# swarth100/dynfu

Hardware: AMD Instinct MI355X
Metric: frames/sec (warp-solve + TSDF fuse), 512^3 vol / 2k nodes / VGA depth (higher is better)
Workload: dtype f32; 1 GPU; C2: 512^3 TSDF, 640x480 depth, 2048 nodes, k=4, 262144 vertices, 5 GN x PCG<=256 (tol 1e-6), reference-parity energy (energy.t), lambda=200; parallelism=replicas x1 (one sequence per GPU, no collective), ranks_seen=1, repeats=5

## Files before the change

dynfu_amd/csrc/capi.cpp:

```cpp
#include <hip/hip_runtime.h>

#include <cmath>
#include <cstdarg>
#include <cstdio>
#include <cstring>
#include <map>
#include <mutex>
#include <new>
#include <utility>
#include <vector>

#include "../../include/dynfu_amd.h"
#include "kernels.hpp"
#include "dev_switch.hpp"
#include "solve.hpp"
#include "solve6.hpp"

namespace {

thread_local char g_err[512] = "";

int fail(int code, const char* fmt, ...) {
    va_list ap;
    va_start(ap, fmt);
// ... 555 lines not shown
int dfa_marching_cubes(const uint32_t* volume, int X, int Y, int Z, const float cell_size[3],
                       const int32_t* tri_table, const int32_t* num_verts_table, float* out_points, int max_vertices,
                       int32_t* total_vertices, dfa_stream_t stream) {
    return marching_cubes_common(volume, X, Y, Z, cell_size, tri_table, num_verts_table, out_points, max_vertices,
                                 total_vertices, nullptr, stream);
}

int dfa_marching_cubes_occ(const uint32_t* volume, const uint8_t* occupancy, int X, int Y, int Z, const float cell_size[3],
                           const int32_t* tri_table, const int32_t* num_verts_table, float* out_points, int max_vertices,
                           int32_t* total_vertices, dfa_stream_t stream) {
    REQUIRE(occupancy, "null occupancy map");
    return marching_cubes_common(volume, X, Y, Z, cell_size, tri_table, num_verts_table, out_points, max_vertices,
                                 total_vertices, occupancy, stream);
}

int dfa_marching_cubes_indexed(const uint32_t* volume, const uint8_t* occupancy, int X, int Y, int Z, const float cell_size[3],
                               const int32_t* tri_table, const int32_t* num_verts_table, float* out_vertices,
                               int max_vertices, int32_t* out_indices, int max_indices, int32_t* totals,
                               dfa_stream_t stream) {
    REQUIRE(volume && X >= 2 && Y >= 2 && Z >= 2, "bad volume");
    REQUIRE(cell_size && tri_table && num_verts_table, "null parameter block / case tables");
    REQUIRE(max_vertices >= 0 && (max_vertices == 0 || out_vertices), "bad vertex buffer");
    REQUIRE(max_indices >= 0 && (max_indices == 0 || out_indices), "bad index buffer");
    REQUIRE(((uintptr_t)out_vertices & 15) == 0, "out_vertices must be 16-byte aligned");
    REQUIRE(totals, "null totals");
    REQUIRE((long)X * Y * Z / 64 < (1L << 31), "volume too large");
    const long nsegs = dfa::mci_segments(X, Y, Z);
    McIndexedScratch& scratch = stream_scratch<McIndexedScratch>(S(stream));
    HIP_TRY(scratch.reserve(nsegs));
    HIP_TRY(dfa::launch_marching_cubes_indexed(volume, X, Y, Z, cell_size, tri_table, num_verts_table, out_vertices,
                                               max_vertices, out_indices, max_indices, totals, scratch.vert.seg_off,
                                               scratch.idx_off, scratch.vert.chunk_sums, occupancy, S(stream)));
    return DFA_OK;
}


static int extract_cloud_common(const uint32_t* volume, int X, int Y, int Z, const float voxel_size[3],
                                const float vol2world[12], float* out_points, int max_points, int32_t* total_points,
                                const uint8_t* occupancy, dfa_stream_t stream) {
    REQUIRE(volume_args_ok(volume, X, Y, Z), "bad volume");
    REQUIRE(voxel_size && vol2world, "null voxel_size / vol2world");
    REQUIRE(max_points >= 0 && (max_points == 0 || out_points), "bad output buffer");
    REQUIRE(((uintptr_t)out_points & 15) == 0, "out_points must be 16-byte aligned");
    REQUIRE((long)X * Y * Z / 64 < (1L << 31), "volume too large");
    const bool vec4  = (X % 4 == 0) && (((uintptr_t)volume & 15) == 0);
    McScratch& scratch = stream_scratch<McScratch>(S(stream));
    HIP_TRY(scratch.reserve(dfa::mc_segments(X, Y, Z, vec4)));
    HIP_TRY(dfa::launch_extract_cloud(volume, X, Y, Z, voxel_size, vol2world, out_points, max_points, total_points,
                                      scratch.seg_off, scratch.chunk_sums, occupancy, S(stream)));
    return DFA_OK;
}

int dfa_tsdf_extract_cloud(const uint32_t* volume, int X, int Y, int Z, const float voxel_size[3], const float vol2world[12],
                           float* out_points, int max_points, int32_t* total_points, dfa_stream_t stream) {
    return extract_cloud_common(volume, X, Y, Z, voxel_size, vol2world, out_points, max_points, total_points, nullptr, stream);
}

int dfa_tsdf_extract_cloud_occ(const uint32_t* volume, const uint8_t* occupancy, int X, int Y, int Z,
                               const float voxel_size[3], const float vol2world[12], float* out_points, int max_points,
                               int32_t* total_points, dfa_stream_t stream) {
    REQUIRE(occupancy, "null occupancy map");
    return extract_cloud_common(volume, X, Y, Z, voxel_size, vol2world, out_points, max_points, total_points, occupancy,
                                stream);
}

int dfa_tsdf_extract_normals(const uint32_t* volume, int X, int Y, int Z, const float voxel_size[3], const float vol2world[12],
                             const float Rinv[9], float gradient_delta_factor, const float* points, int n, float* normals,
                             dfa_stream_t stream) {
    REQUIRE(volume_args_ok(volume, X, Y, Z), "bad volume");
    REQUIRE(voxel_size && vol2world && Rinv, "null voxel_size / vol2world / Rinv");
    REQUIRE(n >= 0 && (n == 0 || (points && normals)), "null points / normals");
    REQUIRE(voxel_size[0] > 0.f && voxel_size[1] > 0.f && voxel_size[2] > 0.f && gradient_delta_factor > 0.f,
            "voxel size and gradient delta must be positive");
    REQUIRE((((uintptr_t)points | (uintptr_t)normals) & 15) == 0, "points / normals must be 16-byte aligned");
    HIP_TRY(dfa::launch_extract_normals(volume, X, Y, Z, voxel_size, vol2world, Rinv, gradient_delta_factor, points, n,
                                        normals, S(stream)));
    return DFA_OK;
}

int dfa_mc_default_tables(int32_t* tri_table, int32_t* num_verts_table) {
    REQUIRE(tri_table && num_verts_table, "null table");
    dfa::mc_default_tables(tri_table, num_verts_table);
    return DFA_OK;
}


int dfa_knn(const float* node_pos, const float* node_w, int D, const float* query, int n_query, int k, int32_t* idx,
            float* weights, dfa_stream_t stream) {
    REQUIRE(node_pos && D > 0, "no nodes");
    REQUIRE(n_query >= 0 && (n_query == 0 || (query && idx)), "bad query / output");
    REQUIRE(k >= 1 && k <= DFA_MAX_KNN, "k out of range 1..16");
    REQUIRE(!weights || node_w, "weights requested without node_w");
    const dfa::KnnGridView* grid = nullptr;
    if (want_grid(D, n_query)) {
        GridScratch& gs = stream_scratch<GridScratch>(S(stream));

        HIP_TRY(gs.reserve(D));

        HIP_TRY(dfa::knn_grid_build(gs.v, node_pos, D, S(stream)));

        grid = &gs.v;
    }
    HIP_TRY(dfa::launch_knn(node_pos, node_w, D, query, n_query, k, idx, weights, grid, S(stream)));
    return DFA_OK;
}

int dfa_warp_to_live(const float* node_pos, const float* node_dq, const float* node_w, int D, int k,
                     const float* vertices, const float* normals, int N, float* out_vertices, float* out_normals,
                     dfa_stream_t stream) {
    REQUIRE(node_pos && node_dq && node_w && D > 0, "no nodes");
    REQUIRE(N >= 0 && (N == 0 || (vertices && out_vertices)), "bad vertices / output");
    REQUIRE(k >= 1 && k <= DFA_MAX_KNN, "k out of range 1..16");
    const dfa::KnnGridView* grid = nullptr;
    if (want_grid(D, N)) {
        GridScratch& gs = stream_scratch<GridScratch>(S(stream));

        HIP_TRY(gs.reserve(D));

        HIP_TRY(dfa::knn_grid_build(gs.v, node_pos, D, S(stream)));

        grid = &gs.v;
    }
    HIP_TRY(dfa::launch_warp_to_live(node_pos, node_dq, node_w, D, k, vertices, normals, N, out_vertices,
                                     out_normals, grid, S(stream)));
    return DFA_OK;
}

int dfa_warp_to_live_graph(const float* node_pos, const float* node_dq, const float* node_w, int D, int k,
                           const int32_t* idx, const float* vertices, const float* normals, int N, float* out_vertices,
                           float* out_normals, dfa_stream_t stream) {
    REQUIRE(node_pos && node_dq && node_w && D > 0, "no nodes");
    REQUIRE(N >= 0 && (N == 0 || (vertices && out_vertices && idx)), "bad vertices / graph / output");
    REQUIRE(k >= 1 && k <= DFA_MAX_KNN, "k out of range 1..16");
    if (N > 0)
        HIP_TRY(dfa::launch_warp_graph(node_pos, node_dq, node_w, k, idx, vertices, normals, N, out_vertices, out_normals,
                                       S(stream)));
    return DFA_OK;
}

int dfa_calc_dqb(const float* node_pos, const float* node_dq, const float* node_w, int D, int k, const float* points,
                 int n, float* out_dq, dfa_stream_t stream) {
    REQUIRE(node_pos && node_dq && node_w && D > 0, "no nodes");
    REQUIRE(n >= 0 && (n == 0 || (points && out_dq)), "bad points / output");
    REQUIRE(k >= 1 && k <= DFA_MAX_KNN, "k out of range 1..16");
    const dfa::KnnGridView* grid = nullptr;
    if (want_grid(D, n)) {
        GridScratch& gs = stream_scratch<GridScratch>(S(stream));

        HIP_TRY(gs.reserve(D));

        HIP_TRY(dfa::knn_grid_build(gs.v, node_pos, D, S(stream)));

        grid = &gs.v;
    }
    HIP_TRY(dfa::launch_dqb_support(node_pos, node_dq, node_w, D, k, points, n, out_dq, nullptr, grid, S(stream)));
    return DFA_OK;
}

int dfa_unsupported_vertices(const float* node_pos, const float* node_w, int D, int k, const float* vertices, int N,
                             uint8_t* flags, dfa_stream_t stream) {
    REQUIRE(N >= 0 && (N == 0 || (vertices && flags)), "bad vertices / output");
    REQUIRE(k >= 1 && k <= DFA_MAX_KNN, "k out of range 1..16");
    if (D == 0) {
        if (N > 0) HIP_TRY(hipMemsetAsync(flags, 1, (size_t)N, S(stream)));
        return DFA_OK;
    }
    REQUIRE(node_pos && node_w && D > 0, "bad nodes");
    const dfa::KnnGridView* grid = nullptr;
    if (want_grid(D, N)) {
        GridScratch& gs = stream_scratch<GridScratch>(S(stream));

        HIP_TRY(gs.reserve(D));

        HIP_TRY(dfa::knn_grid_build(gs.v, node_pos, D, S(stream)));

        grid = &gs.v;
    }
    HIP_TRY(dfa::launch_dqb_support(node_pos, nullptr, node_w, D, k, vertices, N, nullptr, flags, grid, S(stream)));
    return DFA_OK;
}

int dfa_repack_points(const float* src, int src_stride, float* dst, int dst_stride, int n, float pad,
                      dfa_stream_t stream) {
    REQUIRE(n >= 0 && (n == 0 || (src && dst)), "bad points");
    REQUIRE(src_stride >= 3 && dst_stride >= 3, "strides are floats per point, >= 3");
    REQUIRE(src_stride != 4 || ((uintptr_t)src & 15) == 0, "float4 source must be 16-byte aligned");
    REQUIRE(dst_stride != 4 || ((uintptr_t)dst & 15) == 0, "float4 destination must be 16-byte aligned");
    HIP_TRY(dfa::launch_repack_points(src, src_stride, dst, dst_stride, n, pad, S(stream)));
    return DFA_OK;
}

int dfa_transform_points(const float* points, int n, const float aff[12], int with_translation, float* out,
                         dfa_stream_t stream) {
    REQUIRE(n >= 0 && (n == 0 || (points && out)), "bad points");
    REQUIRE(aff, "null transform");
    HIP_TRY(dfa::launch_transform_points(points, n, aff, with_translation != 0, out, S(stream)));
    return DFA_OK;
}

namespace {
struct CompactScratch {
    int32_t* chunks = nullptr;
    int cap         = 0;
    hipError_t reserve(int n_needed) {
        if (n_needed <= cap) return hipSuccess;
        const int n = n_needed + n_needed / 4 + 16;
        (void)hipFree(chunks);
        chunks = nullptr, cap = 0;
        hipError_t e = hipMalloc((void**)&chunks, sizeof(int32_t) * (size_t)n);
        if (e == hipSuccess) cap = n;
        return e;
    }
};
}

int dfa_compact_points(const float* points, const uint8_t* flags, int N, float* out_points, int32_t* out_index,
                       int32_t* count, dfa_stream_t stream) {
    REQUIRE(count, "count is required");
    REQUIRE(N >= 0 && (N == 0 || flags), "bad flags");
    REQUIRE(!out_points || points || N == 0, "out_points requested without points");
    CompactScratch& cs = stream_scratch<CompactScratch>(S(stream));
    HIP_TRY(cs.reserve(dfa::compact_chunks(N > 0 ? N : 1)));
    HIP_TRY(dfa::launch_compact_points(points, flags, N, out_points, out_index, count, cs.chunks, S(stream)));
    return DFA_OK;
}

int dfa_correspond(const float* canon_vertices, const float* canon_normals, int n_canon, const float* live_vertices,
                   int n_live, float* out_vertices, float* out_normals, int32_t* out_index, dfa_stream_t stream) {
    REQUIRE(canon_vertices && n_canon > 0, "no canonical vertices");
    REQUIRE(n_live >= 0 && (n_live == 0 || live_vertices), "bad live vertices");
    REQUIRE(!out_normals || canon_normals, "normals requested without canonical normals");
    const dfa::KnnGridView* grid = nullptr;
    if (n_canon >= 16384 && want_grid(n_canon, n_live)) {
        PointGridScratch& pg = stream_scratch<PointGridScratch>(S(stream));
        HIP_TRY(pg.reserve(n_canon));
        HIP_TRY(dfa::point_grid_build(pg.v, canon_vertices, n_canon, S(stream)));
        grid = &pg.v.g;
    } else if (want_grid(n_canon, n_live)) {
        GridScratch& gs = stream_scratch<GridScratch>(S(stream));

        HIP_TRY(gs.reserve(n_canon));

        HIP_TRY(dfa::knn_grid_build(gs.v, canon_vertices, n_canon, S(stream)));

        grid = &gs.v;
    }
    HIP_TRY(dfa::launch_correspond(canon_vertices, canon_normals, n_canon, live_vertices, n_live, out_vertices,
                                   out_normals, out_index, grid, S(stream)));
    return DFA_OK;
}

int dfa_correspond_projective(const float* vertices, const float* normals, int n, const float* vmap, int vmap_step,
                              const float* nmap, int nmap_step, int cols, int rows, float fx, float fy, float cx, float cy,
                              float dist_thresh, float min_cosine, float* out_vertices, float* out_normals,
                              int32_t* out_pixel, dfa_stream_t stream) {
    REQUIRE(n >= 0 && (n == 0 || vertices), "bad vertices");
    REQUIRE(vmap && cols > 0 && rows > 0 && vmap_step >= 16 * cols, "bad vertex map");
    REQUIRE(!nmap || nmap_step >= 16 * cols, "bad normal map pitch");
    REQUIRE(!out_normals || nmap, "normals requested without a normal map");
    REQUIRE(fx > 0.f && fy > 0.f && dist_thresh >= 0.f, "bad intrinsics / threshold");
    REQUIRE(((uintptr_t)vmap & 15) == 0 && (vmap_step & 15) == 0 && ((uintptr_t)nmap & 15) == 0 && (!nmap || (nmap_step & 15) == 0),
            "maps must be 16-byte aligned float4 images");
    HIP_TRY(dfa::launch_correspond_projective(vertices, normals, n, vmap, vmap_step, nmap, nmap_step, cols, rows, fx, fy, cx,
                                              cy, dist_thresh, min_cosine, out_vertices, out_normals, out_pixel,
                                              S(stream)));
    return DFA_OK;
}


int dfa_solver_create(int max_D, int max_N, int k, dfa_solver** out) {
    REQUIRE(out, "null out");
    *out = nullptr;
    REQUIRE(max_D > 0 && max_N >= 0, "bad sizes");
    REQUIRE(k >= 1 && k <= DFA_MAX_KNN, "k out of range 1..16");
    REQUIRE(max_D <= dfa::solve_pcg_max_nodes(), "more nodes than a plan supports (32768)");
    int ndev = 0;
    if (hipGetDeviceCount(&ndev) != hipSuccess || ndev == 0) return fail(DFA_ERR_NO_GPU, "no HIP device");
    dfa_solver* s = new (std::nothrow) dfa_solver();
    REQUIRE(s, "out of host memory");
    s->max_D = max_D, s->max_N = max_N, s->k = k;
    s->max_R       = (size_t)max_N + (size_t)max_D * k;
    s->ell_cap     = 256;
    s->has_problem = false;
    s->timing      = false;
    {
        const char* e    = getenv("DFA_ASSEMBLE_DETERMINISTIC");
        s->deterministic = e && atoi(e) != 0;
    }
    s->ev_used     = 0;
    std::memset(&s->v, 0, sizeof(s->v));
    const size_t R = s->max_R, D = (size_t)max_D;
    int rc = DFA_OK;
#define A(field, count) \
    if (rc == DFA_OK) rc = plan_alloc(s, &s->v.field, (count))
    A(ridx, R * k);
    A(rw, R * k);
    A(rtau, R);
    A(rb, R * 3);
    A(re, R * (size_t)dfa::solve_rec_words(k));
    A(reg_idx, D * k);
    A(blk_hist, D * (dfa::SOLVE_TG_BLOCKS + 1));
    A(node_ptr, D + 1);
    A(node_list, R * k);
    A(ell, D * s->ell_cap);
    A(ell_cnt, D);
    A(diag, D);
    A(g, D * 3);
    A(g_base, D * 3);
    A(t_base, D * 3);
    A(pk_perm, D);
    A(pk_perm2, D);
    A(pk_vals, D * s->ell_cap);
    A(pk_cols, D * s->ell_cap);
    A(mb_x, D);
    A(mb_r, D);
    A(mb_p, D);
    A(mb_s, D);
    A(mb_w, D);
    A(mb_u[0], D);
    A(mb_u[1], D);
    A(mb_m[0], D);
    A(mb_m[1], D);
    A(mb_t[0], D);
    A(mb_t[1], D);
    A(mb_gpart[0], (size_t)dfa::solve_mb_blocks(max_D));
    A(mb_gpart[1], (size_t)dfa::solve_mb_blocks(max_D));
    A(mb_dpart[0], (size_t)dfa::solve_mb_blocks(max_D));
    A(mb_dpart[1], (size_t)dfa::solve_mb_blocks(max_D));
    A(t, D * 3);
    A(huber, D);
    A(node_dq_out, D * 8);
#undef A
    if (rc == DFA_OK) {
        hipError_t e = s->grid.reserve(max_D);
        if (e != hipSuccess) rc = hip_fail(e, "hipMalloc (node grid)");
    }
    if (rc == DFA_OK && dfa::solve_team_pcg_fits(max_D) && (max_D > 2048 || dfa::kDevAB)) {
        s->v.team_stride = (max_D + 3) & ~3;
        rc = plan_alloc(s, &s->v.team_ctl, 1);
        const size_t areas = (size_t)3 * dfa::solve_team_pcg_rounds();
        if (rc == DFA_OK) rc = plan_alloc(s, &s->v.team_mt, areas * s->v.team_stride);
        if (rc == DFA_OK) rc = plan_alloc(s, &s->v.team_words, dfa::solve_team_pcg_words());
        if (rc == DFA_OK && (hipMemset(s->v.team_ctl, 0, sizeof(dfa::TeamCtl)) != hipSuccess ||
                             hipMemset(s->v.team_words, 0, sizeof(unsigned long long) * dfa::solve_team_pcg_words()) != hipSuccess ||
                             hipMemset(s->v.team_mt, 0, sizeof(float2) * areas * (size_t)s->v.team_stride) != hipSuccess))
            rc = fail(DFA_ERR_HIP, "hipMemset (team PCG)");
        if (rc == DFA_OK && hipHostMalloc((void**)&s->team.host_abort, sizeof(int), hipHostMallocDefault) == hipSuccess) {
            *s->team.host_abort = 0;
            s->team.ctl = s->v.team_ctl;
            if (const char* e0 = dfa::dev_env("DFA_MB_TEAM_EPOCH")) s->team.epoch = (unsigned)std::strtoul(e0, nullptr, 0);
        }
    }
    if (rc == DFA_OK) rc = plan_alloc(s, &s->state, 1);
    if (rc == DFA_OK) rc = plan_alloc(s, &s->iters_total, 1);
    if (rc == DFA_OK && hipMemset(s->iters_total, 0, sizeof(long long)) != hipSuccess) rc = DFA_ERR_HIP;
    if (rc == DFA_OK && hipHostMalloc((void**)&s->host_flag, 4 * sizeof(int), hipHostMallocDefault) != hipSuccess) s->host_flag = nullptr;
    if (rc == DFA_OK) rc = plan_alloc(s, &s->cost_partials, std::max<size_t>((R + 255) / 256 + 1, 1024) + 1024);
    if (rc == DFA_OK) rc = plan_alloc(s, &s->ticket, 64);
    if (rc == DFA_OK && hipMemset(s->ticket, 0, 64 * sizeof(unsigned int)) != hipSuccess)
        rc = fail(DFA_ERR_HIP, "hipMemset (ticket)");
    if (rc != DFA_OK) {
        dfa_solver_destroy(s);
        return rc;
    }
    *out = s;
    return DFA_OK;
}

void dfa_solver_destroy(dfa_solver* s) {
    if (!s) return;
    for (void* p : s->blocks) (void)hipFree(p);
    s->grid.release();
    for (hipEvent_t e : s->events) (void)hipEventDestroy(e);
    if (s->host_flag) (void)hipHostFree(s->host_flag);
    if (s->team.host_abort) (void)hipHostFree(s->team.host_abort);
    s->mb_graphs.release();
    delete s;
}

int dfa_solver_set_problem(dfa_solver* s, const float* node_pos, const float* node_dq, const float* node_w, int D,
                           const float* canon_vertices, const float* canon_normals, const float* live_vertices,
                           const float* live_normals, int N, dfa_stream_t stream) {
    (void)canon_normals;
    (void)live_normals;
    REQUIRE(s, "null plan");
    REQUIRE(node_pos && node_dq && node_w && D > 0, "no nodes");
    REQUIRE(N >= 0 && (N == 0 || (canon_vertices && live_vertices)), "bad vertex arrays");
    if (D > s->max_D || N > s->max_N)
        return fail(DFA_ERR_CAPACITY, "dfa_solver_set_problem: D=%d N=%d exceed the plan (max_D=%d max_N=%d)", D, N,
                    s->max_D, s->max_N);
    dfa::SolveView& v = s->v;
    v.N = N, v.D = D, v.k = s->k, v.Dpad = (D + 3) & ~3, v.ell_cap = s->ell_cap;
    v.deterministic = s->deterministic ? 1 : 0;
    v.node_pos = node_pos, v.node_dq = node_dq, v.node_w = node_w;
    v.canon = canon_vertices, v.live = live_vertices;
    hipStream_t st = S(stream);
    const dfa::KnnGridView* grid = nullptr;
    if (want_grid(D, (long)N + D)) {
        HIP_TRY(dfa::knn_grid_build(s->grid.v, node_pos, D, st));
        grid = &s->grid.v;
    }
    if (N > 0) HIP_TRY(dfa::launch_knn(node_pos, node_w, D, canon_vertices, N, s->k, v.ridx, v.rw, grid, st));
    HIP_TRY(dfa::launch_knn(node_pos, node_w, D, node_pos, D, s->k, v.reg_idx, nullptr, grid, st));
    HIP_TRY(dfa::solve_build_graph(v, s->state, s->ticket, 64, st));
    s->has_problem = true;
    s->just_reset  = true;
    return DFA_OK;
}

int dfa_solver_set_deterministic(dfa_solver* s, int on) {
    REQUIRE(s, "null plan");
    s->deterministic = on != 0;
    return DFA_OK;
}

int dfa_solver_solve(dfa_solver* s, const dfa_solve_params* p, dfa_stream_t stream) {
    REQUIRE(s && p, "null plan / params");
    REQUIRE(s->has_problem, "set_problem has not been called");
    REQUIRE(p->num_iter >= 0 && p->nonlinear_iter >= 0 && p->linear_iter >= 0, "negative iteration count");
    REQUIRE(p->tukey_offset > 0.f && p->psi_data > 0.f, "tukey_offset / psi_data must be positive");
    REQUIRE(p->lambda >= 0.f && std::isfinite(p->lambda), "lambda must be non-negative and finite");
    const dfa::SolveView& v = s->v;
    hipStream_t st          = S(stream);
    if (!s->just_reset) HIP_TRY(dfa::solve_reset(v, s->state, s->ticket, 64, st));
    s->just_reset = false;
    const double w_reg    = std::sqrt((double)p->lambda / ((double)v.D * (double)v.k));
    const float w_reg_f   = (float)w_reg;
    const float w_reg_sq  = w_reg_f * w_reg_f;
    if (s->timing) s->timed_solves += 1;
    if (s->host_flag) s->host_flag[0] = s->host_flag[1] = 0;
    s->mb_graphs.call = 0;
    int not_launched = 0;
    int gn_launched = 0;
    bool huber_done = false;
    const bool big_budget = (long)p->num_iter * p->nonlinear_iter > 8;
    const bool pcg_async  = dfa::solve_pcg_is_async(v, &s->team, p->linear_iter);
    const bool no_regradient = dfa::dev_env("DFA_NO_REGRADIENT") != nullptr;
    for (int outer = 0; outer < p->num_iter; ++outer) {
        if (s->host_flag && s->host_flag[1] == 2) s->host_flag[1] = 0;
        int gn_in_outer = 0;
        for (int gn = 0; gn < p->nonlinear_iter; ++gn) {
            if (big_budget && gn_in_outer >= 4 && gn_in_outer % 4 == 0 && s->host_flag && !s->host_flag[1] && pcg_async) {
                HIP_TRY(hipMemcpyAsync(&s->host_flag[1], &s->state->converged, sizeof(int), hipMemcpyDeviceToHost, st));
                HIP_TRY(hipStreamSynchronize(st));
            }
            if (s->host_flag && s->host_flag[1]) {
                ++not_launched;
                continue;
            }
            ++gn_in_outer;
            if (gn > 0 && p->gn_tol == 0.f && p->lambda > 0.f && !no_regradient) {
                int evg = s->timing ? timing_begin(s, st) : -1;
                HIP_TRY(dfa::solve_regradient(v, s->state, st));
                timing_end(s, evg, st);
                if (evg >= 0) s->ev_asm.push_back(evg);
                if (s->overlap_fn) s->overlap_fn(s->overlap_user, stream, gn_launched);
                ++gn_launched;
                int evr = s->timing ? timing_begin(s, st) : -1;
                HIP_TRY(dfa::solve_pcg(v, s->state, p->linear_iter, p->pcg_tol, s->host_flag, &s->mb_graphs, &s->team,
                                       evr >= 0 ? s->events[evr + 1] : nullptr, st));
                if (evr >= 0) s->ev_pcg.push_back(evr);
                continue;
            }
            const bool with_huber = gn == 0 && outer == p->num_iter - 1;
            HIP_TRY(dfa::solve_linearise(v, s->state, s->cost_partials, s->ticket, gn == 0, gn == 0 ? 0 : 1,
                                         p->gn_tol, p->tukey_offset, p->psi_data, w_reg_sq, with_huber ? p->psi_reg : 0.f, nullptr, st));
            huber_done |= with_huber;
            int ev = s->timing ? timing_begin(s, st) : -1;
            HIP_TRY(dfa::solve_assemble(v, s->state, gn == 0 && p->nonlinear_iter > 1, w_reg_sq, st));
            timing_end(s, ev, st);
            if (ev >= 0) s->ev_asm.push_back(ev);
            if (s->overlap_fn) s->overlap_fn(s->overlap_user, stream, gn_launched);
            ++gn_launched;
            ev = s->timing ? timing_begin(s, st) : -1;
            HIP_TRY(dfa::solve_pcg(v, s->state, p->linear_iter, p->pcg_tol, s->host_flag, &s->mb_graphs, &s->team,
                                   ev >= 0 ? s->events[ev + 1] : nullptr, st));
            if (ev >= 0) s->ev_pcg.push_back(ev);
        }
    }
    if (s->overlap_fn && gn_launched == 0) s->overlap_fn(s->overlap_user, stream, -1);
    if (not_launched) HIP_TRY(dfa::solve_count_noop(s->state, not_launched, st));
    const bool no_weights = p->num_iter == 0 || p->nonlinear_iter == 0;
    if (!huber_done) HIP_TRY(dfa::solve_huber(v, p->psi_reg, st));
    HIP_TRY(dfa::solve_linearise(v, s->state, s->cost_partials, s->ticket, no_weights ? 1 : 0, 2, 0.f,
                                 p->tukey_offset, p->psi_data, w_reg_sq, 0.f, s->timing ? s->iters_total : nullptr, st));
    return DFA_OK;
}

int dfa_solver_set_overlap_callback(dfa_solver* s, dfa_overlap_fn fn, void* user) {
    REQUIRE(s, "null plan");
    s->overlap_fn = fn, s->overlap_user = user;
    return DFA_OK;
}

const float* dfa_solver_translations(const dfa_solver* s) { return s ? s->v.t : nullptr; }
const float* dfa_solver_node_dq(const dfa_solver* s) { return s ? s->v.node_dq_out : nullptr; }
const float* dfa_solver_tukey_weights(const dfa_solver* s) { return s ? s->v.rtau : nullptr; }
const float* dfa_solver_huber_weights(const dfa_solver* s) { return s ? s->v.huber : nullptr; }
const int32_t* dfa_solver_data_graph(const dfa_solver* s) { return s ? s->v.ridx : nullptr; }
const int32_t* dfa_solver_reg_graph(const dfa_solver* s) { return s ? s->v.reg_idx : nullptr; }
const float* dfa_solver_matrix_entries(const dfa_solver* s) { return s ? (const float*)s->v.ell : nullptr; }
const int32_t* dfa_solver_matrix_row_lengths(const dfa_solver* s) { return s ? s->v.ell_cnt : nullptr; }
const float* dfa_solver_gradient(const dfa_solver* s) { return s ? s->v.g : nullptr; }

int dfa_solver_warp_to_live(dfa_solver* s, const float* normals, float* out_vertices, float* out_normals,
                            dfa_stream_t stream) {
    REQUIRE(s && s->has_problem, "no problem set");
    REQUIRE(out_vertices || s->v.N == 0, "null output");
    HIP_TRY(dfa::launch_warp_graph(s->v.node_pos, s->v.node_dq_out, s->v.node_w, s->k, s->v.ridx, s->v.canon, normals,
                                   s->v.N, out_vertices, out_normals, S(stream)));
    return DFA_OK;
}

int dfa_solver_get_stats(dfa_solver* s, dfa_solve_stats* host_out, dfa_stream_t stream) {
    REQUIRE(s && host_out, "null plan / out");
    dfa::SolveState h;
    HIP_TRY(hipMemcpyAsync(&h, s->state, sizeof(h), hipMemcpyDeviceToHost, S(stream)));
    HIP_TRY(hipStreamSynchronize(S(stream)));
    host_out->initial_cost = h.initial_cost;
    host_out->final_cost   = h.final_cost;
    host_out->gn_iters     = h.gn_iters;
    host_out->pcg_iters    = h.pcg_iters;
    host_out->max_row_nnz  = h.max_row_nnz;
    host_out->gn_noop      = h.gn_noop;
    if (dfa::dev_env("DFA_PCG_PROFILE_PRINT"))
        fprintf(stderr, "pcg phase cycles: spmv %lld  red_pAp %lld  update %lld  red_rz %lld  p_update+barrier %lld  loop %lld  (iters %d)\n",
                h.prof[0], h.prof[1], h.prof[2], h.prof[3], h.prof[4], h.prof[5], h.pcg_iters);
    if (dfa::dev_env("DFA_PCG_PROFILE_PRINT"))
        fprintf(stderr, "assemble block 7 cycles: init %lld  list+hash %lld  reduce+barrier %lld  compact %lld   (raw prof[6] %lld prof[7] %lld)\n",
                h.prof[6] / 1000000, h.prof[6] % 1000000, h.prof[7] / 1000000, h.prof[7] % 1000000, h.prof[6], h.prof[7]);
    if (h.overflow)
        return fail(DFA_ERR_CAPACITY, "normal-matrix row wider than the plan's ELL capacity (%d > %d)", h.max_row_nnz,
                    s->ell_cap);
    return DFA_OK;
}

int dfa_solver_enable_timing(dfa_solver* s, int enable) {
    REQUIRE(s, "null plan");
    s->timing = enable != 0;
    if (enable == 1) {
        s->ev_used = 0, s->timed_solves = 0;
        s->ev_pcg.clear(), s->ev_asm.clear();
        if (s->iters_total) HIP_TRY(hipMemset(s->iters_total, 0, sizeof(long long)));
    }
    return DFA_OK;
}

int dfa_solver_team_pcg_info(dfa_solver* s, int* launches, int* aborts, int* disabled) {
    REQUIRE(s, "null plan");
    if (launches) *launches = (int)std::min<long>(s->team.launches, 0x7fffffffL);
    if (aborts) *aborts = s->team.host_abort ? *(volatile int*)s->team.host_abort : 0;
    if (disabled) *disabled = (!s->team.ctl || s->team.disabled) ? 1 : 0;
    return DFA_OK;
}

int dfa_solver_get_timing(dfa_solver* s, dfa_solve_timing* out, dfa_stream_t stream) {
    REQUIRE(s && out, "null plan / out");
    HIP_TRY(hipStreamSynchronize(S(stream)));
    std::memset(out, 0, sizeof(*out));
    for (int idx : s->ev_pcg) {
        float ms = 0.f;
        HIP_TRY(hipEventElapsedTime(&ms, s->events[idx], s->events[idx + 1]));
        out->pcg_ms += ms;
    }
    for (int idx : s->ev_asm) {
        float ms = 0.f;
        HIP_TRY(hipEventElapsedTime(&ms, s->events[idx], s->events[idx + 1]));
        out->assemble_ms += ms;
    }
    out->pcg_launches      = (int)s->ev_pcg.size();
    out->assemble_launches = (int)s->ev_asm.size();
    out->solves            = s->timed_solves;
    if (s->iters_total) HIP_TRY(hipMemcpy(&out->pcg_iters, s->iters_total, sizeof(long long), hipMemcpyDeviceToHost));
    if (s->has_problem && s->v.D > 0) {
        std::vector<int32_t> cnt((size_t)s->v.D);
        HIP_TRY(hipMemcpy(cnt.data(), s->v.ell_cnt, sizeof(int32_t) * cnt.size(), hipMemcpyDeviceToHost));
        long long nnz = 0;
        for (int32_t c : cnt) nnz += c;
        out->matrix_nnz = nnz;
    }
    return DFA_OK;
}


int dfa_compute_points_normals(const uint16_t* depth, int depth_step, int cols, int rows, float fx, float fy, float cx,
                               float cy, float* points, int points_step, float* normals, int normals_step,
                               dfa_stream_t stream) {
    REQUIRE(depth && points && normals && cols > 0 && rows > 0, "bad images");
    REQUIRE(depth_step >= cols * 2 && points_step >= cols * 16 && normals_step >= cols * 16, "row step smaller than a row");
    REQUIRE(fx != 0.f && fy != 0.f, "zero focal length");
    HIP_TRY(dfa::launch_points_normals(depth, depth_step, cols, rows, fx, fy, cx, cy, points, points_step, normals,
                                       normals_step, S(stream)));
    return DFA_OK;
}

int dfa_solver6_create(int max_D, int max_N, int k, dfa_solver6** out) {
    REQUIRE(out, "null out");
    *out = nullptr;
    REQUIRE(max_D > 0 && max_N >= 0, "bad sizes");
    REQUIRE(k >= 1 && k <= 8, "k out of range 1..8");
    int ndev = 0;
    if (hipGetDeviceCount(&ndev) != hipSuccess || ndev == 0) return fail(DFA_ERR_NO_GPU, "no HIP device");
    dfa_solver6* s = new (std::nothrow) dfa_solver6();
    REQUIRE(s, "out of host memory");
    s->max_D = max_D, s->max_N = max_N, s->k = k, s->has_problem = false, s->node_dq = nullptr;
    std::memset(&s->v, 0, sizeof(s->v));
    s->v.cap = DFA_SOLVE6_ROW_BLOCKS;
    const size_t N = (size_t)max_N, D = (size_t)max_D, cap = (size_t)s->v.cap;
    int rc = DFA_OK;
#define A(field, count) \
    if (rc == DFA_OK) rc = plan6_alloc(s, &s->v.field, (count))
    A(idx, N * k);
    A(wn, N * k);
    A(idx_nat, N * k);
    A(near, N);
    A(vptr, D + 1);
    A(vlist, N);
    A(vperm, N);
    A(canon_own, N * 3);
    A(canon_n_own, N * 3);
    A(reg_idx, D * k);
    A(blk_hist, D * (dfa::SOLVE_TG_BLOCKS + 1));
    A(node_ptr, D + 1);
    A(node_list, N * k + 1);
    A(rnode_ptr, D + 1);
    A(rnode_list, D * k + 1);
    A(dq, D * 8);
    A(dq_prev, D * 8);
    A(ghat, D * 3);
    A(rec, N * (12 + (k <= 4 ? 4 : 8)));
    A(cost_part, (N + 255) / 256 + (D * k + 255) / 256 + 1);
    A(valid_part, (N + 255) / 256 + (D * k + 255) / 256 + 1);
    A(mnode, D * 48);
    A(rho, N);
    A(rres, D * k * 3);
    A(rvec, D * k * 18);
    A(rhub, D * k);
    A(bcols, D * cap);
    A(bcnt, D);
    A(bfu, D);
    A(rslot, D * cap);
    A(utab, D * 256);
    A(eslot, N * k * k);
    A(pair_list, N * k * k);
    A(pair_ptr, D * (cap + 1));
    A(bvals, D * cap * 36);
    A(minv, D * 36);
    A(g, D * 6);
    A(x, D * 6);
    A(r, D * 6);
    A(p, D * 6);
    A(s, D * 6);
    A(w, D * 6);
    A(u[0], D * 6);
    A(u[1], D * 6);
    A(t[0], D * 6);
    A(t[1], D * 6);
    A(m[0], D * 6);
    A(m[1], D * 6);
    A(g_part[0], (size_t)dfa::s6_matvec_blocks(max_D));
// ... 280 lines not shown
```

dynfu_amd/csrc/solve.hip:

```cpp
#include <hip/hip_runtime.h>
#include <cstring>

#include <algorithm>
#include <map>
#include <mutex>

#include <float.h>

#include "dq_device.hpp"
#include "dev_switch.hpp"
#include "kernels.hpp"
#include "pcg_rules.hpp"
#include "solve.hpp"

namespace dfa {


constexpr int TG_BLOCKS = SOLVE_TG_BLOCKS;

__global__ __launch_bounds__(1024) void tg_count_kernel(const int32_t* __restrict__ ridx, size_t total, int D,
                                                        int32_t* __restrict__ blk_hist ) {
    extern __shared__ int32_t hist[];
    for (int i = threadIdx.x; i < D; i += blockDim.x) hist[i] = 0;
    __syncthreads();
    const size_t chunk = (total + TG_BLOCKS - 1) / TG_BLOCKS;
    const size_t beg = chunk * blockIdx.x, end = min(beg + chunk, total);
    for (size_t e = beg + threadIdx.x; e < end; e += blockDim.x) {
        const int n = ridx[e];
        if (n >= 0) atomicAdd(&hist[n], 1);
    }
    __syncthreads();
    for (int i = threadIdx.x; i < D; i += blockDim.x) blk_hist[(size_t)blockIdx.x * D + i] = hist[i];
}

__global__ __launch_bounds__(256) void tg_colscan_kernel(int32_t* __restrict__ blk_hist , int D) {
    const int i = blockIdx.x * blockDim.x + threadIdx.x;
    if (i >= D) return;
    constexpr int G = 32;
    static_assert(TG_BLOCKS % G == 0, "workgroups of the counting sort in groups");
    int run = 0;
    for (int b0 = 0; b0 < TG_BLOCKS; b0 += G) {
        int h[G];
#pragma unroll
        for (int b = 0; b < G; ++b) h[b] = blk_hist[(size_t)(b0 + b) * D + i];
#pragma unroll
        for (int b = 0; b < G; ++b) {
            blk_hist[(size_t)(b0 + b) * D + i] = run;
            run += h[b];
        }
    }
    blk_hist[(size_t)TG_BLOCKS * D + i] = run;
}

__global__ __launch_bounds__(1024) void tg_fill_kernel(const int32_t* __restrict__ ridx, size_t total, int D,
                                                       const int32_t* __restrict__ blk_base ,
                                                       int32_t* __restrict__ node_ptr, uint32_t* __restrict__ node_list) {
    extern __shared__ int32_t cursor[];
    __shared__ int32_t wave_tot[16];
    __shared__ int32_t carry_sh;
    const int lane = threadIdx.x & 63, wave = threadIdx.x >> 6;
    if (threadIdx.x == 0) carry_sh = 0;
    __syncthreads();
    for (int base = 0; base < D; base += 1024) {
        const int i = base + threadIdx.x;
        const int v = i < D ? blk_base[(size_t)TG_BLOCKS * D + i] : 0;
        const int incl = wave_inclusive_scan(v);
        if (lane == 63) wave_tot[wave] = incl;
        __syncthreads();
        int off = carry_sh + incl - v;
        for (int w = 0; w < wave; ++w) off += wave_tot[w];
        if (i < D) {
            cursor[i] = off + blk_base[(size_t)blockIdx.x * D + i];
            if (blockIdx.x == 0) node_ptr[i] = off;
        }
        __syncthreads();
        if (threadIdx.x == 1023) carry_sh = off + v;
        __syncthreads();
    }
    if (blockIdx.x == 0 && threadIdx.x == 0) node_ptr[D] = carry_sh;
    const size_t chunk = (total + TG_BLOCKS - 1) / TG_BLOCKS;
    const size_t beg = chunk * blockIdx.x, end = min(beg + chunk, total);
    for (size_t e = beg + threadIdx.x; e < end; e += blockDim.x) {
        const int n = ridx[e];
        if (n >= 0) node_list[atomicAdd(&cursor[n], 1)] = (uint32_t)e;
    }
}


template <int K>
__device__ __forceinline__ void load_row_graph(const SolveView& s, size_t r, int (&n)[K], float (&w)[K]) {
    if (s.k == K) {
#pragma unroll
        for (int q = 0; q < K / 4; ++q) {
            const int4 iv   = reinterpret_cast<const int4*>(s.ridx + r * K)[q];
            const float4 wv = reinterpret_cast<const float4*>(s.rw + r * K)[q];
            n[4 * q] = iv.x, n[4 * q + 1] = iv.y, n[4 * q + 2] = iv.z, n[4 * q + 3] = iv.w;
            w[4 * q] = wv.x, w[4 * q + 1] = wv.y, w[4 * q + 2] = wv.z, w[4 * q + 3] = wv.w;
        }
    } else {
#pragma unroll
        for (int j = 0; j < K; ++j) n[j] = j < s.k ? s.ridx[r * s.k + j] : -1, w[j] = j < s.k ? s.rw[r * s.k + j] : 0.f;
    }
}

template <int K>
__device__ __forceinline__ float tukey_weight(const SolveView& s, size_t v, float tukey_offset, float psi_data) {
    const f3 c = mk3(s.canon[3 * v], s.canon[3 * v + 1], s.canon[3 * v + 2]);
    DQ sum     = dq_identity();
    int n[K];
    float w[K];
    load_row_graph<K>(s, v, n, w);
#pragma unroll
    for (int h = 0; h < K; h += 4) {
        float tx[4], ty[4], tz[4];
        DQ q[4];
#pragma unroll
        for (int jj = 0; jj < 4; ++jj) {
            const int nn = n[h + jj] >= 0 ? n[h + jj] : 0;
            tx[jj] = s.t[3 * nn], ty[jj] = s.t[3 * nn + 1], tz[jj] = s.t[3 * nn + 2];
            q[jj]  = dq_load(s.node_dq + 8 * (size_t)nn);
        }
#pragma unroll
        for (int jj = 0; jj < 4; ++jj) {
            if (n[h + jj] >= 0) {
                const DQ cur = dq_mul(dq_from_translation(tx[jj], ty[jj], tz[jj]), q[jj]);
                sum          = dq_mul(sum, dq_scale(cur, w[h + jj]));
            }
        }
    }
    const f3 warped = dq_transform(dq_normalize(sum), c);
    const float ex = s.live[3 * v] - warped.x, ey = s.live[3 * v + 1] - warped.y, ez = s.live[3 * v + 2] - warped.z;
    const float d = sqrtf(ex * ex + ey * ey + ez * ez) / tukey_offset;
    if (d < psi_data) {
        const double q = 1.0 - ((double)d * (double)d) / ((double)psi_data * (double)psi_data);
        return (float)(q * q);
    }
    return 0.f;
}

__device__ __forceinline__ void huber_node(const SolveView& s, int i, float psi_reg) {
    const DQ dq_i = dq_mul(dq_from_translation(s.t[3 * i], s.t[3 * i + 1], s.t[3 * i + 2]),
                           dq_load(s.node_dq + 8 * (size_t)i));
    float h = 0.f;
    for (int j = 0; j < s.k; ++j) {
        const int m = s.reg_idx[(size_t)i * s.k + j];
        if (m < 0) break;
        const f3 pm   = mk3(s.node_pos[3 * m], s.node_pos[3 * m + 1], s.node_pos[3 * m + 2]);
        const DQ dq_m = dq_mul(dq_from_translation(s.t[3 * m], s.t[3 * m + 1], s.t[3 * m + 2]),
                               dq_load(s.node_dq + 8 * (size_t)m));
        const f3 pa = dq_transform(dq_i, pm), pb = dq_transform(dq_m, pm);
        const float ex = pa.x - pb.x, ey = pa.y - pb.y, ez = pa.z - pb.z;
        const float err = sqrtf(ex * ex + ey * ey + ez * ez);
        h               = fabsf(err) <= psi_reg ? 1.f : psi_reg / fabsf(err);
    }
    s.huber[i] = h;
}
__global__ __launch_bounds__(256) void huber_kernel(SolveView s, float psi_reg) {
    const int i = blockIdx.x * blockDim.x + threadIdx.x;
    if (i < s.D) huber_node(s, i, psi_reg);
}

struct LineariseArgs {
    int update_weights;
    int mode;
    float gn_tol, tukey_offset, psi_data, w_reg_sq;
    long long* iters_total;
    float huber_psi;
};

constexpr int LIN_SHARDS     = 32;
constexpr int LIN_MAX_BLOCKS = 1024;

template <int K>
__global__ __launch_bounds__(256) void linearise_kernel(SolveView s, SolveState* __restrict__ st,
                                                        double* __restrict__ cost_partials,
                                                        unsigned int* __restrict__ ticket ,
                                                        LineariseArgs a) {
    __shared__ double wsum[4];
    __shared__ int is_last;
    if (a.huber_psi > 0.f)
        for (int i = blockIdx.x * blockDim.x + threadIdx.x; i < s.D; i += gridDim.x * blockDim.x) huber_node(s, i, a.huber_psi);
    if (a.mode == 2) {
        for (int i = blockIdx.x * blockDim.x + threadIdx.x; i < s.D; i += gridDim.x * blockDim.x) {
            const DQ out = dq_mul(dq_from_translation(s.t[3 * i], s.t[3 * i + 1], s.t[3 * i + 2]),
                                  dq_load(s.node_dq + 8 * (size_t)i));
            dq_store(s.node_dq_out + 8 * (size_t)i, out);
        }
        if (blockIdx.x == 0 && threadIdx.x == 0 && a.iters_total) *a.iters_total += st->pcg_iters;
    }
    if (st->converged == 1 || (st->converged && !a.update_weights)) {
        if (a.mode != 2 || (st->have_initial && !st->cost_stale)) return;
    }
    const size_t R = (size_t)s.N + (size_t)s.D * s.k;
    double c       = 0.0;
    float amax     = 0.f;
    for (size_t r = (size_t)blockIdx.x * blockDim.x + threadIdx.x; r < R; r += (size_t)gridDim.x * blockDim.x) {
        float tau;
        if (a.update_weights) {
            tau       = r < (size_t)s.N ? tukey_weight<K>(s, r, a.tukey_offset, a.psi_data) : a.w_reg_sq;
            s.rtau[r] = tau;
        } else {
            tau = s.rtau[r];
        }
        float sx = 0.f, sy = 0.f, sz = 0.f;
        {
            int n[K];
            float w[K], tx[K], ty[K], tz[K];
            load_row_graph<K>(s, r, n, w);
#pragma unroll
            for (int j = 0; j < K; ++j) {
                const int nn = n[j] >= 0 ? n[j] : 0;
                tx[j] = s.t[3 * nn], ty[j] = s.t[3 * nn + 1], tz[j] = s.t[3 * nn + 2];
            }
            float wm = 0.f;
#pragma unroll
            for (int j = 0; j < K; ++j)
                if (n[j] >= 0) sx += w[j] * tx[j], sy += w[j] * ty[j], sz += w[j] * tz[j], wm = fmaxf(wm, fabsf(w[j]));
            amax = fmaxf(amax, tau * wm * wm);
        }
        const float ex = s.rb[3 * r] - sx, ey = s.rb[3 * r + 1] - sy, ez = s.rb[3 * r + 2] - sz;
        *(float4*)(s.re + r * (size_t)solve_rec_words(s.k) + solve_rec_tail(s.k)) = make_float4(ex, ey, ez, tau);
        c += (double)tau * ((double)ex * ex + (double)ey * ey + (double)ez * ez);
    }
    c = wave_sum_all(c);
    __shared__ float wmax[4];
#pragma unroll
    for (int o = 32; o > 0; o >>= 1) amax = fmaxf(amax, __shfl_xor(amax, o, 64));
    if ((threadIdx.x & 63) == 0) wsum[threadIdx.x >> 6] = c, wmax[threadIdx.x >> 6] = amax;
    __syncthreads();
    if (threadIdx.x == 0) {
        __hip_atomic_store(&cost_partials[blockIdx.x], (wsum[0] + wsum[1]) + (wsum[2] + wsum[3]), __ATOMIC_RELAXED,
                           __HIP_MEMORY_SCOPE_AGENT);
        if (a.update_weights)
            __hip_atomic_store(&cost_partials[LIN_MAX_BLOCKS + blockIdx.x], (double)fmaxf(fmaxf(wmax[0], wmax[1]), fmaxf(wmax[2], wmax[3])),
                               __ATOMIC_RELAXED, __HIP_MEMORY_SCOPE_AGENT);
        asm volatile("s_waitcnt vmcnt(0)" ::: "memory");
        const unsigned int shard   = blockIdx.x % LIN_SHARDS;
        const unsigned int members = (gridDim.x - shard + LIN_SHARDS - 1) / LIN_SHARDS;
        const unsigned int nshards = min((unsigned int)LIN_SHARDS, gridDim.x);
        int last                   = 0;
        if (__hip_atomic_fetch_add(&ticket[shard], 1u, __ATOMIC_RELAXED, __HIP_MEMORY_SCOPE_AGENT) == members - 1) {
            __hip_atomic_store(&ticket[shard], 0u, __ATOMIC_RELAXED, __HIP_MEMORY_SCOPE_AGENT);
            if (__hip_atomic_fetch_add(&ticket[LIN_SHARDS], 1u, __ATOMIC_RELAXED, __HIP_MEMORY_SCOPE_AGENT) ==
                nshards - 1) {
                __hip_atomic_store(&ticket[LIN_SHARDS], 0u, __ATOMIC_RELAXED, __HIP_MEMORY_SCOPE_AGENT);
                last = 1;
            }
        }
        is_last = last;
    }
    __syncthreads();
    if (!is_last) return;

    __shared__ double sm[256];
    __shared__ double smx[256];
    double acc = 0.0, mx = 0.0;
    {
        constexpr int Q = LIN_MAX_BLOCKS / 256;
        double cq[Q], mq[Q];
#pragma unroll
        for (int q = 0; q < Q; ++q) {
            const unsigned int i = min(threadIdx.x + 256u * q, gridDim.x - 1);
            cq[q] = __hip_atomic_load(&cost_partials[i], __ATOMIC_RELAXED, __HIP_MEMORY_SCOPE_AGENT);
            mq[q] = a.update_weights ? __hip_atomic_load(&cost_partials[LIN_MAX_BLOCKS + i], __ATOMIC_RELAXED, __HIP_MEMORY_SCOPE_AGENT) : 0.0;
        }
#pragma unroll
        for (int q = 0; q < Q; ++q)
            if (threadIdx.x + 256u * q < gridDim.x) acc += cq[q], mx = fmax(mx, mq[q]);
    }
    sm[threadIdx.x] = acc, smx[threadIdx.x] = mx;
    __syncthreads();
    for (int o = 128; o > 0; o >>= 1) {
        if ((int)threadIdx.x < o) sm[threadIdx.x] += sm[threadIdx.x + o], smx[threadIdx.x] = fmax(smx[threadIdx.x], smx[threadIdx.x + o]);
        __syncthreads();
    }
    if (threadIdx.x == 0) {
        const double cost = sm[0];
        if (a.update_weights) st->amax = (float)smx[0];
        if (!st->have_initial) st->initial_cost = cost, st->have_initial = 1;
        if (a.mode == 0) st->done = 0;
        if (a.mode == 1 && !st->done && a.gn_tol > 0.f && (st->cost - cost) <= (double)a.gn_tol * st->cost)
            st->done = 1;
        st->cost       = cost;
        st->final_cost = cost;
        st->cost_stale = 0;
        if (a.mode != 2) st->weights_fresh = a.update_weights;
        if (a.mode != 2 && a.update_weights && st->converged == 2) st->converged = 0;
    }
}

__global__ __launch_bounds__(256) void reset_kernel(float* __restrict__ t, int n3, SolveState* __restrict__ st,
                                                    unsigned int* __restrict__ ticket, int nticket) {
    const int i = blockIdx.x * blockDim.x + threadIdx.x;
    if (i < n3) t[i] = 0.f;
    if (blockIdx.x == 0) {
        unsigned int* w = (unsigned int*)st;
        for (int j = threadIdx.x; j < (int)(sizeof(SolveState) / 4); j += blockDim.x) w[j] = 0u;
        for (int j = threadIdx.x; j < nticket; j += blockDim.x) ticket[j] = 0u;
    }
}

template <int K>
__global__ __launch_bounds__(256) void prepare_rows_kernel(SolveView s, SolveState* __restrict__ st,
                                                           unsigned int* __restrict__ ticket, int nticket) {
    const size_t R = (size_t)s.N + (size_t)s.D * s.k;
    const size_t r = (size_t)blockIdx.x * blockDim.x + threadIdx.x;
    if (r < (size_t)3 * s.D) s.t[r] = 0.f;
    if (blockIdx.x == 0) {
        unsigned int* w = (unsigned int*)st;
        for (int j = threadIdx.x; j < (int)(sizeof(SolveState) / 4); j += blockDim.x) w[j] = 0u;
        for (int j = threadIdx.x; j < nticket; j += blockDim.x) ticket[j] = 0u;
    }
    if (r >= R) return;
    const int k = s.k;
    int ids[K];
    float ws[K];
    const bool wide = k == K && K % 4 == 0;
    if (r < (size_t)s.N) {
#pragma unroll
        for (int c = 0; c < 3; ++c) s.rb[3 * r + c] = s.live[3 * r + c] - s.canon[3 * r + c];
        if (wide) load_row_graph<K>(s, r, ids, ws);
        else {
#pragma unroll
            for (int j = 0; j < K; ++j)
                if (j < k) ids[j] = s.ridx[r * k + j], ws[j] = s.rw[r * k + j];
        }
    } else {
        const int e = (int)(r - (size_t)s.N), n = e / k, m = s.reg_idx[e];
#pragma unroll
        for (int j = 0; j < K; ++j) ids[j] = -1, ws[j] = 0.f;
        if (m >= 0 && m != n) ids[0] = m, ws[0] = -1.f, ids[1] = n, ws[1] = +1.f;
        if (wide) {
#pragma unroll
            for (int q = 0; q < K / 4; ++q) {
                reinterpret_cast<int4*>(s.ridx + r * K)[q]  = make_int4(ids[4 * q], ids[4 * q + 1], ids[4 * q + 2], ids[4 * q + 3]);
                reinterpret_cast<float4*>(s.rw + r * K)[q] = make_float4(ws[4 * q], ws[4 * q + 1], ws[4 * q + 2], ws[4 * q + 3]);
            }
        } else {
#pragma unroll
            for (int j = 0; j < K; ++j)
                if (j < k) s.ridx[r * k + j] = ids[j], s.rw[r * k + j] = ws[j];
        }
        s.rb[3 * r + 0] = s.rb[3 * r + 1] = s.rb[3 * r + 2] = 0.f;
    }
    float* rec = s.re + r * (size_t)solve_rec_words(k);
    if (wide) {
        float4* rec4 = reinterpret_cast<float4*>(rec);
        if (solve_rec_ids16(k)) {
            uint32_t pk[K / 2];
#pragma unroll
            for (int j = 0; j < K / 2; ++j) {
                const uint32_t lo = ids[2 * j] < 0 ? 0xffffu : (uint32_t)ids[2 * j], hi = ids[2 * j + 1] < 0 ? 0xffffu : (uint32_t)ids[2 * j + 1];
                pk[j]             = (lo & 0xffffu) | (hi << 16);
            }
#pragma unroll
            for (int q = 0; q < K / 8; ++q)
                rec4[q] = make_float4(__uint_as_float(pk[4 * q]), __uint_as_float(pk[4 * q + 1]), __uint_as_float(pk[4 * q + 2]), __uint_as_float(pk[4 * q + 3]));
#pragma unroll
            for (int q = 0; q < K / 4; ++q) rec4[K / 8 + q] = make_float4(ws[4 * q], ws[4 * q + 1], ws[4 * q + 2], ws[4 * q + 3]);
        } else {
#pragma unroll
            for (int q = 0; q < K / 4; ++q)
                rec4[q] = make_float4(__int_as_float(ids[4 * q]), __int_as_float(ids[4 * q + 1]), __int_as_float(ids[4 * q + 2]), __int_as_float(ids[4 * q + 3]));
#pragma unroll
            for (int q = 0; q < K / 4; ++q) rec4[K / 4 + q] = make_float4(ws[4 * q], ws[4 * q + 1], ws[4 * q + 2], ws[4 * q + 3]);
        }
        return;
    }
    if (solve_rec_ids16(k)) {
        uint16_t* h = reinterpret_cast<uint16_t*>(rec);
#pragma unroll
        for (int j = 0; j < K; ++j)
            if (j < k) h[j] = ids[j] < 0 ? (uint16_t)0xffffu : (uint16_t)ids[j], rec[k / 2 + j] = ws[j];
        return;
    }
#pragma unroll
    for (int j = 0; j < K; ++j)
        if (j < k) rec[j] = __int_as_float(ids[j]), rec[k + j] = ws[j];
}


constexpr int HASH      = 512;
constexpr int HASH_MASK = HASH - 1;

struct FixedScale {
    float up;
    double down;
};
__device__ __forceinline__ FixedScale solve_fixed_scale(float amax) {
    int e = 0;
    (void)frexpf(fmaxf(amax, 1e-30f), &e);
    e = e < -80 ? -80 : e > 100 ? 100 : e;
    FixedScale f;
    f.up   = ldexpf(1.f, 40 - e);
    f.down = ldexp(1.0, e - 40);
    return f;
}
__device__ __forceinline__ FixedScale fixed_scale_for_rows(FixedScale f, int rows) {
    const int extra = 32 - __clz((unsigned)max(rows, 1) >> 22);
    if (extra > 0) f.up = ldexpf(f.up, -extra), f.down = ldexp(f.down, extra);
    return f;
}
__device__ __forceinline__ void fixed_add(long long* cell, float v, float up) {
    const float x  = truncf(fabsf(v) * up);
    const float hf = floorf(x * 2.3283064365386963e-10f);
    const uint32_t hi = (uint32_t)hf, lo = (uint32_t)fmaf(hf, -4294967296.f, x);
    atomicAdd(reinterpret_cast<unsigned long long*>(v < 0.f ? cell + HASH : cell), ((unsigned long long)hi << 32) | lo);
}

template <int K>
__device__ __forceinline__ float4 load_record(const SolveView& s, size_t r, int (&idx)[K], float (&w)[K]) {
    const float* rec = s.re + r * (size_t)solve_rec_words(s.k);
    if (s.k == K && (K % 8) == 0) {
        const float4* v = (const float4*)rec;
#pragma unroll
        for (int q = 0; q < K / 8; ++q) {
            const float4 i4 = v[q];
            const uint32_t u[4] = {__float_as_uint(i4.x), __float_as_uint(i4.y), __float_as_uint(i4.z), __float_as_uint(i4.w)};
#pragma unroll
            for (int h = 0; h < 4; ++h) {
                const int lo = (int)(u[h] & 0xffffu), hi = (int)(u[h] >> 16);
                idx[8 * q + 2 * h]     = lo == 0xffff ? -1 : lo;
                idx[8 * q + 2 * h + 1] = hi == 0xffff ? -1 : hi;
            }
        }
#pragma unroll
        for (int q = 0; q < K / 4; ++q) {
            const float4 w4 = v[K / 8 + q];
            w[4 * q] = w4.x, w[4 * q + 1] = w4.y, w[4 * q + 2] = w4.z, w[4 * q + 3] = w4.w;
        }
        return v[K / 8 + K / 4];
    }
    if (solve_rec_ids16(s.k)) {
        const uint16_t* ids = reinterpret_cast<const uint16_t*>(rec);
#pragma unroll
        for (int j = 0; j < K; ++j) {
            idx[j] = j < s.k ? (ids[j] == 0xffffu ? -1 : (int)ids[j]) : -1;
            w[j]   = j < s.k ? rec[s.k / 2 + j] : 0.f;
        }
        const float* tl = rec + solve_rec_tail(s.k);
        return make_float4(tl[0], tl[1], tl[2], tl[3]);
    }
    if (s.k == K && (K % 4) == 0) {
        const float4* v = (const float4*)rec;
#pragma unroll
        for (int q = 0; q < K / 4; ++q) {
            const float4 i4 = v[q], w4 = v[K / 4 + q];
            idx[4 * q] = __float_as_int(i4.x), idx[4 * q + 1] = __float_as_int(i4.y);
            idx[4 * q + 2] = __float_as_int(i4.z), idx[4 * q + 3] = __float_as_int(i4.w);
            w[4 * q] = w4.x, w[4 * q + 1] = w4.y, w[4 * q + 2] = w4.z, w[4 * q + 3] = w4.w;
        }
        return v[K / 2];
    }
#pragma unroll
    for (int j = 0; j < K; ++j) {
        idx[j] = j < s.k ? __float_as_int(rec[j]) : -1;
        w[j]   = j < s.k ? rec[s.k + j] : 0.f;
    }
    return make_float4(rec[2 * s.k], rec[2 * s.k + 1], rec[2 * s.k + 2], rec[2 * s.k + 3]);
}

#ifdef DFA_PCG_PROFILE
__device__ unsigned long long asm_tbuf[32768 * 8];
extern "C" __attribute__((visibility("default"))) int dfa_dev_asm_timing(unsigned long long* out, int n) {
    return (int)hipMemcpyFromSymbol(out, HIP_SYMBOL(asm_tbuf), sizeof(unsigned long long) * 8 * (size_t)n);
}
#endif

template <int K>
__global__ __launch_bounds__(256) void assemble_kernel(SolveView s, SolveState* __restrict__ st, int save_base, float amax_unset) {
    __shared__ int key[HASH];
    __shared__ long long val[2 * HASH];
    __shared__ float gpart[4][3];
    __shared__ int wave_cnt[4];
    __shared__ int ovf;
    if (st->done || st->converged) return;
    const int a = blockIdx.x;
    const int wave = threadIdx.x >> 6, lane = threadIdx.x & 63;
#ifdef DFA_PCG_PROFILE
    long long t0_ = clock64(), t1_, t2_, t3_, t4_;
    const unsigned long long w0_ = wall_clock64();
#endif
    for (int i = threadIdx.x; i < HASH; i += 256) key[i] = -1, val[i] = val[i + HASH] = 0ll;
    if (threadIdx.x == 0) ovf = 0;
    __syncthreads();
#ifdef DFA_PCG_PROFILE
    t1_ = clock64();
#endif

    const int beg = s.node_ptr[a], end = s.node_ptr[a + 1];
    const FixedScale fx = fixed_scale_for_rows(solve_fixed_scale(st->amax > 0.f ? st->amax : amax_unset), end - beg);
    float gx = 0.f, gy = 0.f, gz = 0.f, dsum = 0.f;
    for (int p = beg + (int)threadIdx.x; p < end; p += 256) {
        const uint32_t e = s.node_list[p];
        const size_t r   = e / (uint32_t)s.k;
        const int slot   = (int)(e - (uint32_t)r * (uint32_t)s.k);
        int idx[K];
        float w[K];
        const float4 et = load_record<K>(s, r, idx, w);
        float wa = 0.f;
#pragma unroll
        for (int j = 0; j < K; ++j) wa = (j == slot) ? w[j] : wa;
        const float tw = et.w * wa;
        gx += tw * et.x, gy += tw * et.y, gz += tw * et.z;
        if (et.w != 0.f) {
            uint32_t h0[K];
            int k0[K];
#pragma unroll
            for (int j = 0; j < K; ++j) {
                h0[j] = ((uint32_t)idx[j] * 2654435761u) >> (32 - 9);
                k0[j] = key[h0[j]];
            }
#pragma unroll
            for (int j = 0; j < K; ++j) {
                const int b = idx[j];
                if (b < 0) continue;
                const float v = tw * w[j];
                if (b == a) {
                    dsum += v;
                    continue;
                }
                if (k0[j] == b) {
                    fixed_add(&val[h0[j]], v, fx.up);
                    continue;
                }
                uint32_t h = h0[j];
                int cur    = k0[j];
#pragma unroll 1
                for (int probes = 0;; ++probes) {
                    if (cur == -1) cur = atomicCAS(&key[h], -1, b), cur = cur == -1 ? b : cur;
                    if (cur == b) {
                        fixed_add(&val[h], v, fx.up);
                        break;
                    }
                    if (probes >= HASH) {
                        ovf = 1;
                        break;
                    }
                    h   = (h + 1) & HASH_MASK;
                    cur = key[h];
                }
            }
        }
    }
    dsum = wave_total(dsum);
    if (lane == 0 && dsum != 0.f) {
        uint32_t h = ((uint32_t)a * 2654435761u) >> (32 - 9);
        for (int probes = 0; probes < HASH; ++probes, h = (h + 1) & HASH_MASK) {
            const int cur = atomicCAS(&key[h], -1, a);
            if (cur == -1 || cur == a) {
                fixed_add(&val[h], dsum, fx.up);
                break;
            }
        }
    }
#ifdef DFA_PCG_PROFILE
    t2_ = clock64();
#endif
    gx = wave_total(gx), gy = wave_total(gy), gz = wave_total(gz);
    if (lane == 0) gpart[wave][0] = gx, gpart[wave][1] = gy, gpart[wave][2] = gz;
    __syncthreads();
#ifdef DFA_PCG_PROFILE
    t3_ = clock64();
#endif
    constexpr int PER_WAVE = HASH / 4;
    constexpr int PER_LANE = PER_WAVE / 64;
    int kk[PER_LANE];
    float vv[PER_LANE];
    int wcnt = 0;
#pragma unroll
    for (int i = 0; i < PER_LANE; ++i) {
        const int hq = wave * PER_WAVE + 64 * i + lane;
        kk[i]        = key[hq];
        vv[i]        = (float)((double)(val[hq] - val[hq + HASH]) * fx.down);
        wcnt += __popcll(__ballot(kk[i] >= 0));
    }
    if (lane == 0) wave_cnt[wave] = wcnt;
    __syncthreads();
    int pos0 = 0, total = 0;
#pragma unroll
    for (int w = 0; w < 4; ++w) {
        pos0 += w < wave ? wave_cnt[w] : 0;
        total += wave_cnt[w];
    }
#pragma unroll
    for (int i = 0; i < PER_LANE; ++i) {
        const uint64_t m = __ballot(kk[i] >= 0);
        if (kk[i] >= 0) key[pos0 + __popcll(m & ((1ull << lane) - 1ull))] = kk[i];
        pos0 += __popcll(m);
    }
    __syncthreads();
    int rank[PER_LANE] = {};
    for (int q = 0; q < total; ++q) {
        const int kq = key[q];
#pragma unroll
        for (int i = 0; i < PER_LANE; ++i) rank[i] += kq < kk[i];
    }
    float diag = 0.f;
#pragma unroll
    for (int i = 0; i < PER_LANE; ++i) {
        if (kk[i] < 0) continue;
        if (rank[i] < s.ell_cap) s.ell[(size_t)rank[i] * s.D + a] = make_float2(vv[i], __int_as_float(kk[i]));
        if (kk[i] == a) s.diag[a] = vv[i], diag = 1.f;
    }
    const bool has_diag = __syncthreads_or(diag != 0.f);
    if (threadIdx.x == 0) {
        s.ell_cnt[a] = min(total, s.ell_cap);
        if (!has_diag) s.diag[a] = 0.f;
#pragma unroll
        for (int c = 0; c < 3; ++c) {
            const float gc = (gpart[0][c] + gpart[1][c]) + (gpart[2][c] + gpart[3][c]);
            s.g[3 * a + c] = gc;
            if (save_base) s.g_base[3 * a + c] = gc, s.t_base[3 * a + c] = s.t[3 * a + c];
        }
        if (total > *(volatile int*)&st->max_row_nnz) atomicMax(&st->max_row_nnz, total);
        if (total > s.ell_cap || ovf) st->overflow = 1;
#ifdef DFA_PCG_PROFILE
        t4_ = clock64();
        if (a == 7 && !s.team_ctl) st->prof[6] = (t1_ - t0_) * 1000000 + (t2_ - t1_), st->prof[7] = (t3_ - t2_) * 1000000 + (t4_ - t3_);
        if (a < 32768) {
            unsigned long long* o = asm_tbuf + 8 * (size_t)a;
            o[0] = w0_, o[1] = wall_clock64() - w0_, o[2] = (unsigned long long)(end - beg), o[3] = (unsigned long long)total;
            o[4] = t1_ - t0_, o[5] = t2_ - t1_, o[6] = t3_ - t2_, o[7] = t4_ - t3_;
        }
#endif
    }
}

constexpr int DET_SORT_MAX = 4096;

__global__ __launch_bounds__(256) void sort_node_lists_kernel(const int32_t* __restrict__ node_ptr, uint32_t* __restrict__ node_list) {
    __shared__ uint32_t buf[DET_SORT_MAX];
    const int a = blockIdx.x, tid = threadIdx.x;
    const int beg = node_ptr[a], len = node_ptr[a + 1] - beg;
    if (len < 2 || len > DET_SORT_MAX) return;
    int n2 = 1;
    while (n2 < len) n2 <<= 1;
    for (int i = tid; i < n2; i += 256) buf[i] = i < len ? node_list[beg + i] : 0xffffffffu;
    __syncthreads();
    for (int size = 2; size <= n2; size <<= 1)
        for (int stride = size >> 1; stride > 0; stride >>= 1) {
            for (int i = tid; i < n2 / 2; i += 256) {
                const int lo = 2 * i - (i & (stride - 1)), hi = lo + stride;
                const bool up = (lo & size) == 0;
                const uint32_t x = buf[lo], y = buf[hi];
                if ((x > y) == up) buf[lo] = y, buf[hi] = x;
            }
            __syncthreads();
        }
    for (int i = tid; i < len; i += 256) node_list[beg + i] = buf[i];
}

template <int K>
__global__ __launch_bounds__(256) void assemble_det_kernel(SolveView s, SolveState* __restrict__ st, int save_base, float amax_unset) {
    __shared__ int key[HASH];
    __shared__ long long val[2 * HASH];
    __shared__ float gpart[4][3], dpart[4];
    __shared__ int ovf, nkeys;
    if (st->done || st->converged) return;
    const int a    = blockIdx.x;
    const int wave = threadIdx.x >> 6, lane = threadIdx.x & 63;
    for (int i = threadIdx.x; i < HASH; i += 256) key[i] = -1, val[i] = val[i + HASH] = 0ll;
    if (threadIdx.x == 0) ovf = 0, nkeys = 0;
    __syncthreads();
    const int beg = s.node_ptr[a], end = s.node_ptr[a + 1];
    const FixedScale fx = fixed_scale_for_rows(solve_fixed_scale(st->amax > 0.f ? st->amax : amax_unset), end - beg);
    float gx = 0.f, gy = 0.f, gz = 0.f, dsum = 0.f;
    for (int p = beg + (int)threadIdx.x; p < end; p += 256) {
        const uint32_t e = s.node_list[p];
        const size_t r   = e / (uint32_t)s.k;
        const int slot   = (int)(e - (uint32_t)r * (uint32_t)s.k);
        int idx[K];
        float w[K];
        const float4 et = load_record<K>(s, r, idx, w);
        float wa = 0.f;
#pragma unroll
        for (int j = 0; j < K; ++j) wa = (j == slot) ? w[j] : wa;
        const float tw = et.w * wa;
        gx += tw * et.x, gy += tw * et.y, gz += tw * et.z;
        if (et.w != 0.f) {
#pragma unroll
            for (int j = 0; j < K; ++j) {
                const int b = idx[j];
                if (b < 0) continue;
                if (b == a) {
                    dsum += tw * w[j];
                    continue;
                }
                uint32_t h = ((uint32_t)b * 2654435761u) >> (32 - 9);
                for (int probes = 0;; ++probes) {
                    const int cur = atomicCAS(&key[h], -1, b);
                    if (cur == -1 || cur == b) break;
                    if (probes >= HASH) {
                        ovf = 1;
                        break;
                    }
                    h = (h + 1) & HASH_MASK;
                }
            }
        }
    }
    dsum = wave_total(dsum), gx = wave_total(gx), gy = wave_total(gy), gz = wave_total(gz);
    if (lane == 0) dpart[wave] = dsum, gpart[wave][0] = gx, gpart[wave][1] = gy, gpart[wave][2] = gz;
    __syncthreads();
    const float dtot = (dpart[0] + dpart[1]) + (dpart[2] + dpart[3]);
    if (threadIdx.x == 0 && dtot != 0.f) {
        uint32_t h = ((uint32_t)a * 2654435761u) >> (32 - 9);
        for (int probes = 0; probes < HASH; ++probes, h = (h + 1) & HASH_MASK)
            if (key[h] == -1) {
                key[h] = a;
                break;
            }
    }
    __syncthreads();
    for (int p = beg + (int)threadIdx.x; p < end; p += 256) {
        const uint32_t e = s.node_list[p];
        const size_t r   = e / (uint32_t)s.k;
        const int slot   = (int)(e - (uint32_t)r * (uint32_t)s.k);
        int idx[K];
        float w[K];
        const float4 et = load_record<K>(s, r, idx, w);
        if (et.w == 0.f) continue;
        float wa = 0.f;
#pragma unroll
        for (int j = 0; j < K; ++j) wa = (j == slot) ? w[j] : wa;
        const float tw = et.w * wa;
#pragma unroll
        for (int j = 0; j < K; ++j) {
            const int b = idx[j];
            if (b < 0 || b == a) continue;
            uint32_t h = ((uint32_t)b * 2654435761u) >> (32 - 9);
            for (int probes = 0; probes <= HASH && key[h] != b; ++probes) h = (h + 1) & HASH_MASK;
            if (key[h] == b) fixed_add(&val[h], tw * w[j], fx.up);
        }
    }
    __syncthreads();
    int total = 0;
    for (int i = threadIdx.x; i < HASH; i += 256) total += key[i] >= 0;
    total = (int)wave_total((float)total);
    if (lane == 0) atomicAdd(&nkeys, total);
    __syncthreads();
    total = nkeys;
    bool has_diag = false;
    for (int i = threadIdx.x; i < HASH; i += 256) {
        const int kk = key[i];
        if (kk < 0) continue;
        int pos = 0;
        for (int q = 0; q < HASH; ++q) pos += key[q] >= 0 && key[q] < kk;
        const float vv = kk == a ? dtot : (float)((double)(val[i] - val[i + HASH]) * fx.down);
        if (pos < s.ell_cap) s.ell[(size_t)pos * s.D + a] = make_float2(vv, __int_as_float(kk));
        if (kk == a) s.diag[a] = vv, has_diag = true;
    }
    const bool any_diag = __syncthreads_or(has_diag);
    if (threadIdx.x == 0) {
        s.ell_cnt[a] = min(total, s.ell_cap);
        if (!any_diag) s.diag[a] = 0.f;
#pragma unroll
        for (int c = 0; c < 3; ++c) {
            const float gc = (gpart[0][c] + gpart[1][c]) + (gpart[2][c] + gpart[3][c]);
            s.g[3 * a + c] = gc;
            if (save_base) s.g_base[3 * a + c] = gc, s.t_base[3 * a + c] = s.t[3 * a + c];
        }
        if (total > *(volatile int*)&st->max_row_nnz) atomicMax(&st->max_row_nnz, total);
        if (total > s.ell_cap || ovf) st->overflow = 1;
    }
}

template <int NT, int R>
__device__ __forceinline__ void stable_equal_runs(const int32_t* from, int32_t* to, const int32_t* cnt_of_row, const int* hist, int D) {
#pragma unroll
    for (int i = 0; i < R; ++i) {
        const int rank = (int)threadIdx.x + NT * i;
        if (rank >= D) continue;
        const int row = from[rank];
        const int bin = 256 - min(cnt_of_row[row], 256);
        const int beg = bin > 0 ? hist[bin - 1] : 0, end = hist[bin];
        int before = 0;
        for (int q = beg; q < end; ++q) before += from[q] < row;
        to[beg + before] = row;
    }
}


template <int NWAVES>
__device__ __forceinline__ double block_sum(float v, float* red) {
    const float w = wave_total(v);
    if ((threadIdx.x & 63) == 0) red[threadIdx.x >> 6] = w;
    __syncthreads();
    double tot = 0.0;
#pragma unroll
    for (int i = 0; i < NWAVES; ++i) tot += (double)red[i];
    return tot;
}

#ifdef DFA_PCG_PROFILE
#define PROF_MARK(i)                      \
    do {                                  \
        const long long now_ = clock64(); \
        pc_[i] += now_ - last_;           \
        last_ = now_;                     \
    } while (0)
#else
#define PROF_MARK(i)
#endif

template <int NWAVES>
__device__ __forceinline__ float block_sum_f(float v, float* red) {
    const float w = wave_total(v);
    if ((threadIdx.x & 63) == 0) red[threadIdx.x >> 6] = w;
    __syncthreads();
    float tot = 0.f;
#pragma unroll
    for (int i = 0; i < NWAVES; ++i) tot += red[i];
    return tot;
}

template <int NT, int RPT>
__device__ __forceinline__ void pcg_stream_body(const SolveView& s, SolveState* __restrict__ st, int max_iter, float pcg_tol,
                                                char* smem) {
    float4* p_s = (float4*)smem;
    float* red0 = (float*)(smem + sizeof(float4) * (size_t)s.Dpad);
    float* red1 = red0 + 16;
    int* hist   = (int*)(red1 + 16);
    const int tid = threadIdx.x;
    const int D   = s.D;

    for (int i = tid; i < 260; i += NT) hist[i] = 0;
    __syncthreads();
    int my_cnt[RPT];
#pragma unroll
    for (int h = 0; h < RPT; ++h) {
        const int row = tid + NT * h;
        my_cnt[h]     = row < D ? min(s.ell_cnt[row], 256) : -1;
        if (my_cnt[h] >= 0) atomicAdd(&hist[256 - my_cnt[h]], 1);
    }
    __syncthreads();
    if (tid < 64) {
        int loc[5], sum = 0;
#pragma unroll
        for (int j = 0; j < 5; ++j) {
            const int b = tid * 5 + j;
            loc[j]      = b < 257 ? hist[b] : 0;
            sum += loc[j];
        }
        int incl = sum;
#pragma unroll
        for (int o = 1; o < 64; o <<= 1) {
            const int t = __shfl_up(incl, o, 64);
            if (tid >= o) incl += t;
        }
        int off = incl - sum;
#pragma unroll
        for (int j = 0; j < 5; ++j) {
            const int b = tid * 5 + j;
            if (b < 257) hist[b] = off;
            off += loc[j];
        }
    }
    __syncthreads();
#pragma unroll
    for (int h = 0; h < RPT; ++h)
        if (my_cnt[h] >= 0) (s.deterministic ? s.pk_perm2 : s.pk_perm)[atomicAdd(&hist[256 - my_cnt[h]], 1)] = tid + NT * h;
    __syncthreads();
    if (s.deterministic) {
        stable_equal_runs<NT, RPT>(s.pk_perm2, s.pk_perm, s.ell_cnt, hist, D);
        __syncthreads();
    }

    int row[RPT], rcnt[RPT], wmax[RPT];
#pragma unroll
    for (int i = 0; i < RPT; ++i) {
        const int rank = tid + NT * i;
        row[i]         = rank < D ? s.pk_perm[rank] : -1;
        rcnt[i]        = row[i] >= 0 ? min(s.ell_cnt[row[i]], 256) : 0;
        for (int q = 0; q < rcnt[i]; ++q) {
            const float2 e                  = s.ell[(size_t)q * D + row[i]];
            s.pk_vals[(size_t)q * D + rank] = e.x;
            s.pk_cols[(size_t)q * D + rank] = (uint16_t)__float_as_int(e.y);
        }
        int m = rcnt[i];
#pragma unroll
        for (int o = 32; o > 0; o >>= 1) m = max(m, __shfl_xor(m, o, 64));
        wmax[i] = m;
    }
    __syncthreads();

    float x[RPT][3], r[RPT][3], p[RPT][3], minv[RPT];
    float rz_loc = 0.f;
#pragma unroll
    for (int i = 0; i < RPT; ++i) {
        if (row[i] >= 0) {
            minv[i] = jacobi_inv(s.diag[row[i]]);
#pragma unroll
            for (int c = 0; c < 3; ++c) {
                x[i][c] = 0.f;
                r[i][c] = s.g[3 * row[i] + c];
                p[i][c] = minv[i] * r[i][c];
                rz_loc  = fmaf(r[i][c], p[i][c], rz_loc);
            }
            p_s[row[i]] = make_float4(p[i][0], p[i][1], p[i][2], 0.f);
        } else {
            minv[i] = 0.f;
#pragma unroll
            for (int c = 0; c < 3; ++c) x[i][c] = r[i][c] = p[i][c] = 0.f;
        }
    }
    double rz           = block_sum<NT / 64>(rz_loc, red1);
    const double rz0    = rz;
    const double floor_ = 1e-12;
    const double tol2   = (double)pcg_tol * (double)pcg_tol > floor_ ? (double)pcg_tol * (double)pcg_tol : floor_;
    int it              = 0;
    const bool skip     = pcg_at_floor(st, rz0);
    const double target = fmax(tol2 * rz0, (double)solve_floor(st));
    if (!skip) {
        while (it < max_iter) {
            if (!(rz > 0.0)) break;
            float ap[RPT][3];
            float pap_loc = 0.f;
#pragma unroll
            for (int i = 0; i < RPT; ++i) {
                const int rank  = tid + NT * i;
                const int rankc = rank < D ? rank : 0;
                float ax = 0.f, ay = 0.f, az = 0.f;
                for (int q0 = 0; q0 < wmax[i]; q0 += 8) {
                    int colv[8];
                    float valv[8];
#pragma unroll
                    for (int u = 0; u < 8; ++u) {
                        const int q = min(q0 + u, 255);
                        colv[u]     = s.pk_cols[(size_t)q * D + rankc];
                        valv[u]     = s.pk_vals[(size_t)q * D + rankc];
                    }
#pragma unroll
                    for (int u = 0; u < 8; ++u) {
                        const bool ok = q0 + u < rcnt[i];
                        colv[u]       = ok ? colv[u] : 0;
                        valv[u]       = ok ? valv[u] : 0.f;
                    }
#pragma unroll
                    for (int u = 0; u < 8; ++u) {
                        const float4 pc = p_s[colv[u]];
                        ax = fmaf(valv[u], pc.x, ax), ay = fmaf(valv[u], pc.y, ay), az = fmaf(valv[u], pc.z, az);
                    }
                }
                ap[i][0] = ax, ap[i][1] = ay, ap[i][2] = az;
                pap_loc = fmaf(p[i][0], ax, fmaf(p[i][1], ay, fmaf(p[i][2], az, pap_loc)));
            }
            const double pAp = block_sum<NT / 64>(pap_loc, red0);
            if (!(pAp > 0.0)) break;
            const float alpha = (float)(rz / pAp);
            float rzn_loc     = 0.f;
#pragma unroll
            for (int i = 0; i < RPT; ++i) {
#pragma unroll
                for (int c = 0; c < 3; ++c) {
                    x[i][c] = fmaf(alpha, p[i][c], x[i][c]);
                    r[i][c] = fmaf(-alpha, ap[i][c], r[i][c]);
                    rzn_loc = fmaf(r[i][c], minv[i] * r[i][c], rzn_loc);
                }
            }
            const double rz_new = block_sum<NT / 64>(rzn_loc, red1);
            ++it;
            if (rz_new <= target) break;
            const float beta = (float)(rz_new / rz);
#pragma unroll
            for (int i = 0; i < RPT; ++i) {
#pragma unroll
                for (int c = 0; c < 3; ++c) p[i][c] = fmaf(beta, p[i][c], minv[i] * r[i][c]);
                if (row[i] >= 0) p_s[row[i]] = make_float4(p[i][0], p[i][1], p[i][2], 0.f);
            }
            rz = rz_new;
            __syncthreads();
        }
    }
#pragma unroll
    for (int i = 0; i < RPT; ++i) {
        if (row[i] >= 0) {
#pragma unroll
            for (int c = 0; c < 3; ++c) s.t[3 * row[i] + c] += x[i][c];
        }
    }
    if (tid == 0) pcg_book_launch(st, rz0, it, skip);
}

template <int NT, int E, int NC>
__global__ __launch_bounds__(NT) void pcg_paired_kernel(SolveView s, SolveState* __restrict__ st, int max_iter,
                                                        float pcg_tol) {
    extern __shared__ __attribute__((aligned(16))) char smem[];
    const int D     = s.D;
    const int c0    = NC == 1 ? (int)blockIdx.x : 0;
    float4* p_s     = (float4*)smem;
    float* p_s1     = (float*)smem;
    float* red0     = (float*)(smem + sizeof(float4) * (size_t)s.Dpad);
    float* red1     = red0 + 16;
    int* hist       = (int*)(red1 + 16);
    int* perm       = hist + 260;
    if (st->done) return;
    const int tid = threadIdx.x;
    if (st->converged) {
        if (tid == 0 && blockIdx.x == 0) st->gn_iters += 1, st->gn_noop += 1;
        return;
    }
    constexpr int P = 1;
    constexpr int R = 2 * P;

    float rzj_loc = 0.f;
#pragma unroll
    for (int h = 0; h < R; ++h) {
        const int row = tid + NT * h;
        if (row < D) {
            const float minv = jacobi_inv(s.diag[row]);
#pragma unroll
            for (int c = 0; c < 3; ++c) {
                const float g = s.g[3 * row + c];
                rzj_loc       = fmaf(g, minv * g, rzj_loc);
            }
        }
    }
    const float rz0 = block_sum_f<NT / 64>(rzj_loc, red1);
    const bool skip = pcg_at_floor(st, rz0);
    if (skip) {
        if (tid == 0 && blockIdx.x == 0) {
            st->gn_iters += 1;
            solve_mark_at_floor(st);
        }
        return;
    }

    for (int i = tid; i < 260; i += NT) hist[i] = 0;
    __syncthreads();
    int my_cnt[R];
#pragma unroll
    for (int h = 0; h < R; ++h) {
        const int row = tid + NT * h;
        my_cnt[h]     = row < D ? min(s.ell_cnt[row], 256) : -1;
        if (my_cnt[h] >= 0) atomicAdd(&hist[256 - my_cnt[h]], 1);
    }
    __syncthreads();
    if (tid < 64) {
        int loc[5], sum = 0;
#pragma unroll
        for (int j = 0; j < 5; ++j) {
            const int b = tid * 5 + j;
            loc[j]      = b < 257 ? hist[b] : 0;
            sum += loc[j];
        }
        int incl = sum;
#pragma unroll
        for (int o = 1; o < 64; o <<= 1) {
            const int t = __shfl_up(incl, o, 64);
            if (tid >= o) incl += t;
        }
        int off = incl - sum;
#pragma unroll
        for (int j = 0; j < 5; ++j) {
            const int b = tid * 5 + j;
            if (b < 257) hist[b] = off;
            off += loc[j];
        }
    }
    __syncthreads();
#pragma unroll
    for (int h = 0; h < R; ++h)
        if (my_cnt[h] >= 0) (s.deterministic ? perm + s.Dpad : perm)[atomicAdd(&hist[256 - my_cnt[h]], 1)] = tid + NT * h;
    __syncthreads();
    if (s.deterministic) {
        stable_equal_runs<NT, R>(perm + s.Dpad, perm, s.ell_cnt, hist, D);
        __syncthreads();
    }
// ... 2 lines not shown
    bool unfit_any = false;
#pragma unroll
    for (int j = 0; j < P; ++j) {
        const int ia = j * NT + tid, ib = D - 1 - j * NT - tid;
        rowA[j]      = (ia < D && ia <= ib) ? perm[ia] : -1;
        rowB[j]      = (ib >= 0 && ib > ia) ? perm[ib] : -1;
        const int cntA = rowA[j] >= 0 ? min(s.ell_cnt[rowA[j]], 256) : 0;
        const int cntB = rowB[j] >= 0 ? min(s.ell_cnt[rowB[j]], 256) : 0;
        cntA_[j] = cntA, cntB_[j] = cntB;
        int na         = min(cntA, E);
#pragma unroll
        for (int o = 32; o > 0; o >>= 1) na = max(na, __shfl_xor(na, o, 64));
        na             = (na + 1) & ~1;
        const int capB = E - na;
        const int regB = min(cntB, capB);
        int nb         = regB;
#pragma unroll
        for (int o = 32; o > 0; o >>= 1) nb = max(nb, __shfl_xor(nb, o, 64));
        nA[j] = __builtin_amdgcn_readfirstlane(na), nB[j] = __builtin_amdgcn_readfirstlane(min((nb + 1) & ~1, capB));
        unfit_any |= cntA > E || cntB > capB;
    }
    if (__syncthreads_or(unfit_any)) {
        if (NC == 3 || blockIdx.x == 0) pcg_stream_body<NT, 2 * P>(s, st, max_iter, pcg_tol, smem);
        return;
    }
    float mval[P][E];
    uint32_t mcol[P][E / 2];
#pragma unroll
    for (int j = 0; j < P; ++j) {
        const int cntA = cntA_[j], cntB = cntB_[j];
        const int na = nA[j];
        const int regB = min(cntB, E - na);
        const int rA = rowA[j] >= 0 ? rowA[j] : 0, rB = rowB[j] >= 0 ? rowB[j] : 0;
#pragma unroll
        for (int q2 = 0; q2 < E / 2; ++q2) {
            uint32_t packed = 0;
#pragma unroll
            for (int h = 0; h < 2; ++h) {
                const int q     = 2 * q2 + h;
                const bool isA  = q < na;
                const int ent   = isA ? q : E - 1 - q;
                const int r     = isA ? rA : rB;
                const bool live = isA ? (q < cntA) : (E - 1 - q < regB);
                const float2 e  = s.ell[(size_t)ent * D + r];
                float v         = e.x;
                int col         = __float_as_int(e.y);
                if (!live) v = 0.f, col = 0;
                mval[j][q] = v;
                packed |= (uint32_t)(col << (NC == 3 ? 4 : 2)) << (16 * h);
            }
            mcol[j][q2] = packed;
            if ((q2 & 3) == 3) __builtin_amdgcn_sched_barrier(0);
        }
    }
    float xA[P][NC], rA_[P][NC], pA[P][NC], xB[P][NC], rB_[P][NC], pB[P][NC], minvA[P], minvB[P];
#pragma unroll
    for (int j = 0; j < P; ++j) {
        minvA[j] = minvB[j] = 0.f;
        if (rowA[j] >= 0) minvA[j] = jacobi_inv(s.diag[rowA[j]]);
        if (rowB[j] >= 0) minvB[j] = jacobi_inv(s.diag[rowB[j]]);
#pragma unroll
        for (int cc = 0; cc < NC; ++cc) {
            const int c    = c0 + cc;
            const float ga = rowA[j] >= 0 ? s.g[3 * rowA[j] + c] : 0.f;
            const float gb = rowB[j] >= 0 ? s.g[3 * rowB[j] + c] : 0.f;
            xA[j][cc] = xB[j][cc] = 0.f;
            rA_[j][cc] = ga, rB_[j][cc] = gb;
            pA[j][cc] = minvA[j] * ga, pB[j][cc] = minvB[j] * gb;
        }
        if (NC == 3) {
            if (rowA[j] >= 0) p_s[rowA[j]] = make_float4(pA[j][0], pA[j][1], pA[j][NC - 1], 0.f);
            if (rowB[j] >= 0) p_s[rowB[j]] = make_float4(pB[j][0], pB[j][1], pB[j][NC - 1], 0.f);
        } else {
            if (rowA[j] >= 0) p_s1[rowA[j]] = pA[j][0];
            if (rowB[j] >= 0) p_s1[rowB[j]] = pB[j][0];
        }
    }
    __syncthreads();
    float rz = rz0;
    const float joint  = pcg_joint_target(st, pcg_tol, rz0);
    const float target = NC == 3 ? joint : joint * (1.0f / 3.0f);
    int it             = 0;
    const char* pbase   = (const char*)p_s;
#ifdef DFA_PCG_PROFILE
    long long pc_[6] = {0, 0, 0, 0, 0, 0};
    long long last_  = clock64();
#endif
    auto matvec = [&](float (&aA)[P][NC], float (&aB)[P][NC]) __attribute__((always_inline)) {
#pragma unroll
        for (int j = 0; j < P; ++j) {
#pragma unroll
            for (int c = 0; c < NC; ++c) aA[j][c] = aB[j][c] = 0.f;
            auto slots2 = [&](const int q, float (&acc)[NC]) __attribute__((always_inline)) {
                uint32_t cw = mcol[j][q / 2];
                asm volatile("" : "+v"(cw));
                const float v0 = mval[j][q], v1 = mval[j][q + 1];
                if (NC == 3) {
                    const float4 g0 = *(const float4*)(pbase + (cw & 0xffffu));
                    const float4 g1 = *(const float4*)(pbase + (cw >> 16));
                    asm volatile("" ::"v"(g0.w), "v"(g1.w));
                    acc[0]      = fmaf(v1, g1.x, fmaf(v0, g0.x, acc[0]));
                    acc[NC / 2] = fmaf(v1, g1.y, fmaf(v0, g0.y, acc[NC / 2]));
                    acc[NC - 1] = fmaf(v1, g1.z, fmaf(v0, g0.z, acc[NC - 1]));
                } else {
                    const float g0 = *(const float*)(pbase + (cw & 0xffffu));
                    const float g1 = *(const float*)(pbase + (cw >> 16));
                    acc[0]         = fmaf(v1, g1, fmaf(v0, g0, acc[0]));
                }
            };
            auto slots4 = [&](const int q, float (&acc)[NC]) __attribute__((always_inline)) {
                uint32_t c01 = mcol[j][q / 2], c23 = mcol[j][q / 2 + 1];
                asm volatile("" : "+v"(c01), "+v"(c23));
                const float v0 = mval[j][q], v1 = mval[j][q + 1], v2 = mval[j][q + 2], v3 = mval[j][q + 3];
                if (NC == 3) {
                    const float4 g0 = *(const float4*)(pbase + (c01 & 0xffffu));
                    const float4 g1 = *(const float4*)(pbase + (c01 >> 16));
                    const float4 g2 = *(const float4*)(pbase + (c23 & 0xffffu));
                    const float4 g3 = *(const float4*)(pbase + (c23 >> 16));
                    asm volatile("" ::"v"(g0.w), "v"(g1.w), "v"(g2.w), "v"(g3.w));
                    acc[0]      = fmaf(v3, g3.x, fmaf(v2, g2.x, fmaf(v1, g1.x, fmaf(v0, g0.x, acc[0]))));
                    acc[NC / 2] = fmaf(v3, g3.y, fmaf(v2, g2.y, fmaf(v1, g1.y, fmaf(v0, g0.y, acc[NC / 2]))));
                    acc[NC - 1] = fmaf(v3, g3.z, fmaf(v2, g2.z, fmaf(v1, g1.z, fmaf(v0, g0.z, acc[NC - 1]))));
                } else {
                    const float g0 = *(const float*)(pbase + (c01 & 0xffffu));
                    const float g1 = *(const float*)(pbase + (c01 >> 16));
                    const float g2 = *(const float*)(pbase + (c23 & 0xffffu));
                    const float g3 = *(const float*)(pbase + (c23 >> 16));
                    acc[0]         = fmaf(v3, g3, fmaf(v2, g2, fmaf(v1, g1, fmaf(v0, g0, acc[0]))));
                }
            };
#pragma unroll
            for (int q0 = 0; q0 < E; q0 += 4) {
                if (q0 + 4 <= nA[j]) {
                    slots4(q0, aA[j]);
                } else {
                    if (q0 + 2 <= nA[j]) slots2(q0, aA[j]);
                    break;
                }
            }
#pragma unroll
            for (int q0 = E - 4; q0 >= 0; q0 -= 4) {
                if (q0 >= E - nB[j]) {
                    slots4(q0, aB[j]);
                } else {
                    if (q0 + 2 >= E - nB[j]) slots2(q0 + 2, aB[j]);
                    break;
                }
            }
        }
    };
    auto publish = [&](const float (&vA)[P][NC], const float (&vB)[P][NC]) __attribute__((always_inline)) {
#pragma unroll
        for (int j = 0; j < P; ++j) {
            if (NC == 3) {
                if (rowA[j] >= 0) p_s[rowA[j]] = make_float4(vA[j][0], vA[j][NC / 2], vA[j][NC - 1], 0.f);
                if (rowB[j] >= 0) p_s[rowB[j]] = make_float4(vB[j][0], vB[j][NC / 2], vB[j][NC - 1], 0.f);
            } else {
                if (rowA[j] >= 0) p_s1[rowA[j]] = vA[j][0];
                if (rowB[j] >= 0) p_s1[rowB[j]] = vB[j][0];
            }
        }
    };
    if (NC == 3) {
        while (it < max_iter) {
            if (!(rz > 0.f)) break;
            PROF_MARK(5);
            float aA[P][NC], aB[P][NC];
            float pap_loc = 0.f;
            matvec(aA, aB);
#pragma unroll
            for (int j = 0; j < P; ++j)
#pragma unroll
                for (int c = 0; c < NC; ++c) pap_loc = fmaf(pA[j][c], aA[j][c], fmaf(pB[j][c], aB[j][c], pap_loc));
            PROF_MARK(0);
            const float pAp = block_sum_f<NT / 64>(pap_loc, red0);
            PROF_MARK(1);
            if (!(pAp > 0.f)) break;
            const float alpha = rz / pAp;
            float rzn_loc     = 0.f;
#pragma unroll
            for (int j = 0; j < P; ++j)
#pragma unroll
                for (int c = 0; c < NC; ++c) {
                    xA[j][c]  = fmaf(alpha, pA[j][c], xA[j][c]);
                    xB[j][c]  = fmaf(alpha, pB[j][c], xB[j][c]);
                    rA_[j][c] = fmaf(-alpha, aA[j][c], rA_[j][c]);
                    rB_[j][c] = fmaf(-alpha, aB[j][c], rB_[j][c]);
                    rzn_loc = fmaf(rA_[j][c], minvA[j] * rA_[j][c], fmaf(rB_[j][c], minvB[j] * rB_[j][c], rzn_loc));
                }
            PROF_MARK(2);
            const float rz_new = block_sum_f<NT / 64>(rzn_loc, red1);
            PROF_MARK(3);
            ++it;
            if (rz_new <= target) break;
            const float beta = rz_new / rz;
#pragma unroll
            for (int j = 0; j < P; ++j)
#pragma unroll
                for (int c = 0; c < NC; ++c) {
                    pA[j][c] = fmaf(beta, pA[j][c], minvA[j] * rA_[j][c]);
                    pB[j][c] = fmaf(beta, pB[j][c], minvB[j] * rB_[j][c]);
                }
            publish(pA, pB);
            rz = rz_new;
            __syncthreads();
            PROF_MARK(4);
        }
    }
    if (NC == 1) {
        float sA[P][NC], sB[P][NC], uA[P][NC], uB[P][NC];
#pragma unroll
        for (int j = 0; j < P; ++j)
#pragma unroll
            for (int c = 0; c < NC; ++c) {
                uA[j][c] = pA[j][c], uB[j][c] = pB[j][c];
                pA[j][c] = pB[j][c] = sA[j][c] = sB[j][c] = 0.f;
            }
        float gamma_old = 1.f, alpha_old = 1.f;
        __syncthreads();
        while (it < max_iter) {
            PROF_MARK(5);
            float wA[P][NC], wB[P][NC];
            matvec(wA, wB);
            float g_loc = 0.f, d_loc = 0.f;
#pragma unroll
            for (int j = 0; j < P; ++j)
#pragma unroll
                for (int c = 0; c < NC; ++c) {
                    g_loc = fmaf(rA_[j][c], uA[j][c], fmaf(rB_[j][c], uB[j][c], g_loc));
                    d_loc = fmaf(wA[j][c], uA[j][c], fmaf(wB[j][c], uB[j][c], d_loc));
                }
            PROF_MARK(0);
            const float gw = wave_total(g_loc), dw = wave_total(d_loc);
            if ((tid & 63) == 0) red0[tid >> 6] = gw, red1[tid >> 6] = dw;
            __syncthreads();
            float gamma = 0.f, delta = 0.f;
#pragma unroll
            for (int i = 0; i < NT / 64; ++i) gamma += red0[i], delta += red1[i];
            PROF_MARK(1);
            if (!(gamma > target)) break;
            const float beta  = cg_beta(it == 0, gamma, gamma_old);
            const float denom = cg_denom(it == 0, gamma, delta, beta, alpha_old);
            if (!(denom > 0.f)) break;
            const float alpha = gamma / denom;
#pragma unroll
            for (int j = 0; j < P; ++j)
#pragma unroll
                for (int c = 0; c < NC; ++c) {
                    cg_update_row(alpha, beta, uA[j][c], wA[j][c], pA[j][c], sA[j][c], xA[j][c], rA_[j][c]);
                    cg_update_row(alpha, beta, uB[j][c], wB[j][c], pB[j][c], sB[j][c], xB[j][c], rB_[j][c]);
                    uA[j][c]  = minvA[j] * rA_[j][c];
                    uB[j][c]  = minvB[j] * rB_[j][c];
                }
            ++it;
            gamma_old = gamma, alpha_old = alpha;
            PROF_MARK(2);
            publish(uA, uB);
            __syncthreads();
            PROF_MARK(4);
        }
    }
#ifdef DFA_PCG_PROFILE
    if (tid == 0 && c0 == 0)
        for (int i = 0; i < 6; ++i) st->prof[i] += pc_[i];
#endif
#pragma unroll
    for (int j = 0; j < P; ++j)
#pragma unroll
        for (int c = 0; c < NC; ++c) {
            if (rowA[j] >= 0) s.t[3 * rowA[j] + c0 + c] += xA[j][c];
            if (rowB[j] >= 0) s.t[3 * rowB[j] + c0 + c] += xB[j][c];
        }
    if (tid == 0) {
        if (NC == 3) pcg_book_launch(st, rz0, it, false);
        else pcg_book_launch_of_three(st, rz0, it, false);
    }
}


#define KDISPATCH(kernel, k, ...)                      \
    do {                                               \
        if ((k) <= 4) kernel<4> __VA_ARGS__;           \
        else if ((k) <= 8) kernel<8> __VA_ARGS__;      \
        else kernel<16> __VA_ARGS__;                   \
    } while (0)

hipError_t solve_transpose_graph(const int32_t* ridx, size_t total, int D, int32_t* blk_hist, int32_t* node_ptr,
                                 uint32_t* node_list, hipStream_t st) {
    const size_t lds = sizeof(int32_t) * (size_t)D;
    tg_count_kernel<<<TG_BLOCKS, 1024, lds, st>>>(ridx, total, D, blk_hist);
    tg_colscan_kernel<<<(D + 255) / 256, 256, 0, st>>>(blk_hist, D);
    tg_fill_kernel<<<TG_BLOCKS, 1024, lds, st>>>(ridx, total, D, blk_hist, node_ptr, node_list);
    return hipGetLastError();
}

hipError_t solve_build_graph(const SolveView& s, SolveState* state, unsigned int* ticket, int nticket, hipStream_t st) {
    const int D = s.D, N = s.N, k = s.k;
    const size_t R = (size_t)N + (size_t)D * k, total = R * k;
    const size_t threads = R > (size_t)3 * D ? R : (size_t)3 * D;
    KDISPATCH(prepare_rows_kernel, k, <<<(unsigned)((threads + 255) / 256), 256, 0, st>>>(s, state, ticket, nticket));
    const size_t lds = sizeof(int32_t) * (size_t)D;
    tg_count_kernel<<<TG_BLOCKS, 1024, lds, st>>>(s.ridx, total, D, s.blk_hist);
    tg_colscan_kernel<<<(D + 255) / 256, 256, 0, st>>>(s.blk_hist, D);
    tg_fill_kernel<<<TG_BLOCKS, 1024, lds, st>>>(s.ridx, total, D, s.blk_hist, s.node_ptr, s.node_list);
    if (s.deterministic) sort_node_lists_kernel<<<D, 256, 0, st>>>(s.node_ptr, s.node_list);
    return hipGetLastError();
}

int solve_residual_blocks(const SolveView& s) {
    const size_t R  = (size_t)s.N + (size_t)s.D * s.k;
    const size_t nb = (R + 255) / 256;
    return (int)(nb < (size_t)LIN_MAX_BLOCKS ? nb : (size_t)LIN_MAX_BLOCKS);
}

hipError_t solve_linearise(const SolveView& s, SolveState* state, double* cost_partials, unsigned int* ticket,
                           int update_weights, int mode, float gn_tol, float tukey_offset, float psi_data,
                           float w_reg_sq, float huber_psi, long long* iters_total, hipStream_t st) {
    const int nb = solve_residual_blocks(s);
    LineariseArgs a{update_weights, mode, gn_tol, tukey_offset, psi_data, w_reg_sq, iters_total, huber_psi};
    KDISPATCH(linearise_kernel, s.k, <<<nb, 256, 0, st>>>(s, state, cost_partials, ticket, a));
    return hipGetLastError();
}

hipError_t solve_reset(const SolveView& s, SolveState* state, unsigned int* ticket, int nticket, hipStream_t st) {
    reset_kernel<<<(3 * s.D + 255) / 256, 256, 0, st>>>(s.t, 3 * s.D, state, ticket, nticket);
    return hipGetLastError();
}

hipError_t solve_huber(const SolveView& s, float psi_reg, hipStream_t st) {
    huber_kernel<<<(s.D + 255) / 256, 256, 0, st>>>(s, psi_reg);
    return hipGetLastError();
}

hipError_t solve_assemble(const SolveView& s, SolveState* state, int save_base, float w_reg_sq, hipStream_t st) {
    const float amax_unset = std::max(1.0f, w_reg_sq);
    if (s.deterministic) KDISPATCH(assemble_det_kernel, s.k, <<<s.D, 256, 0, st>>>(s, state, save_base, amax_unset));
    else KDISPATCH(assemble_kernel, s.k, <<<s.D, 256, 0, st>>>(s, state, save_base, amax_unset));
    return hipGetLastError();
}

__global__ __launch_bounds__(256) void regradient_kernel(SolveView s, SolveState* __restrict__ st) {
    if (st->done || st->converged) return;
    const int a = blockIdx.x * blockDim.x + threadIdx.x;
    if (a == 0) st->cost_stale = 1, st->weights_fresh = 0;
    if (a >= s.D) return;
    const int cnt = s.ell_cnt[a];
    float sx = 0.f, sy = 0.f, sz = 0.f;
    for (int q = 0; q < cnt; ++q) {
        const float2 e = s.ell[(size_t)q * s.D + a];
        const int col  = __float_as_int(e.y);
        sx = fmaf(e.x, s.t[3 * col] - s.t_base[3 * col], sx);
        sy = fmaf(e.x, s.t[3 * col + 1] - s.t_base[3 * col + 1], sy);
        sz = fmaf(e.x, s.t[3 * col + 2] - s.t_base[3 * col + 2], sz);
    }
    s.g[3 * a] = s.g_base[3 * a] - sx, s.g[3 * a + 1] = s.g_base[3 * a + 1] - sy, s.g[3 * a + 2] = s.g_base[3 * a + 2] - sz;
}

hipError_t solve_regradient(const SolveView& s, SolveState* state, hipStream_t st) {
    regradient_kernel<<<(s.D + 255) / 256, 256, 0, st>>>(s, state);
    return hipGetLastError();
}

constexpr int MB_LPR = 16;

__device__ __forceinline__ float sum_partials_mb(const float* __restrict__ part, int n) {
    float acc = 0.f;
    for (int i = threadIdx.x & 63; i < n; i += 64) acc += part[i];
    return wave_sum_all(acc);
}

__global__ __launch_bounds__(256) void pcg_mb_init_kernel(SolveView s, SolveState* __restrict__ st) {
    __shared__ float sh[4];
    const int a = blockIdx.x * blockDim.x + threadIdx.x;
    if (a == 0) {
        st->mb_done = st->done || st->converged ? 1 : 0, st->mb_skip = st->done ? 1 : 0, st->mb_iters = 0, st->mb_rz0 = 0.f;
        if (st->converged) st->gn_noop += 1;
    }
    float rz = 0.f;
    if (a < s.D) {
        const float minv = jacobi_inv(s.diag[a]);
        const float4 r   = make_float4(s.g[3 * a], s.g[3 * a + 1], s.g[3 * a + 2], 0.f);
        const float4 z   = make_float4(minv * r.x, minv * r.y, minv * r.z, 0.f);
        const float4 zero = make_float4(0.f, 0.f, 0.f, 0.f);
        s.mb_r[a] = r, s.mb_u[0][a] = z, s.mb_x[a] = zero;
        s.mb_p[a] = s.mb_s[a] = s.mb_t[0][a] = s.mb_t[1][a] = zero;
        rz = fmaf(r.z, z.z, fmaf(r.y, z.y, r.x * z.x));
    }
    rz = wave_sum_all(rz);
    if ((threadIdx.x & 63) == 0) sh[threadIdx.x >> 6] = rz;
    __syncthreads();
    if (threadIdx.x == 0) s.mb_gpart[0][blockIdx.x] = (sh[0] + sh[1]) + (sh[2] + sh[3]);
}

__device__ __forceinline__ float group16_sum(float v) {
#pragma unroll
    for (int o = 8; o > 0; o >>= 1) v += __shfl_xor(v, o, 64);
    return v;
}

__global__ __launch_bounds__(256) void pcg_mb_step_kernel(SolveView s, SolveState* __restrict__ st, int it, float pcg_tol) {
    __shared__ float sh[2][4];
    const int nb  = solve_mb_blocks(s.D);
    const int cur = it >= 0 ? (it & 1) : 0, nxt = cur ^ 1;
    const float4* ucur  = s.mb_u[cur];
    const float4* mcur  = s.mb_m[cur];
    const float4* tprev = s.mb_t[nxt];
    const int lane16  = threadIdx.x & (MB_LPR - 1);
    const int a       = (blockIdx.x * 256 + threadIdx.x) / MB_LPR;
    const bool row_ok = a < s.D;
    const int cnt     = row_ok ? s.ell_cnt[a] : 0;
    const float2 e0   = row_ok ? s.ell[(size_t)lane16 * s.D + a] : make_float2(0.f, 0.f);
    const float2 e1   = row_ok ? s.ell[(size_t)(lane16 + MB_LPR) * s.D + a] : make_float2(0.f, 0.f);
    if (st->mb_done) return;
    const bool has0 = lane16 < cnt, has1 = lane16 + MB_LPR < cnt;
    const int col0  = has0 ? __float_as_int(e0.y) : 0, col1 = has1 ? __float_as_int(e1.y) : 0;
    const float4 uu0 = ucur[col0], uu1 = ucur[col1];
    float4 mm0 = make_float4(0.f, 0.f, 0.f, 0.f), tt0 = mm0, mm1 = mm0, tt1 = mm0;
    if (it >= 0) mm0 = mcur[col0], tt0 = tprev[col0], mm1 = mcur[col1], tt1 = tprev[col1];
    float alpha = 0.f, beta = 0.f;
    if (it >= 0) {
        float g = 0.f, d = 0.f;
        for (int i = threadIdx.x; i < nb; i += 256) g += s.mb_gpart[it & 1][i], d += s.mb_dpart[it & 1][i];
        g = wave_sum_all(g), d = wave_sum_all(d);
        if ((threadIdx.x & 63) == 0) sh[0][threadIdx.x >> 6] = g, sh[1][threadIdx.x >> 6] = d;
        __syncthreads();
        const float gamma = (sh[0][0] + sh[0][1]) + (sh[0][2] + sh[0][3]), delta = (sh[1][0] + sh[1][1]) + (sh[1][2] + sh[1][3]);
        float denom = delta;
        bool stop   = !(gamma > 0.f);
        if (it == 0) {
            const bool at_floor = pcg_at_floor(st, gamma, (double)1e-12f);
            stop                = stop || at_floor;
            if (blockIdx.x == 0 && threadIdx.x == 0) {
                st->mb_rz0 = gamma;
                if (at_floor) solve_mark_at_floor(st);
            }
        } else {
            beta  = cg_beta(false, gamma, st->mb_gamma_prev[(it + 1) & 1]);
            denom = cg_denom(false, gamma, delta, beta, st->mb_alpha_prev[(it + 1) & 1]);
            stop  = stop || gamma <= pcg_joint_target(st, pcg_tol, st->mb_rz0);
        }
        stop = stop || !(denom > 0.f);
        if (stop) {
            if (blockIdx.x == 0 && threadIdx.x == 0) st->mb_done = 1;
            return;
        }
        alpha = gamma / denom;
        if (blockIdx.x == 0 && threadIdx.x == 0) {
            st->mb_gamma_prev[it & 1] = gamma, st->mb_alpha_prev[it & 1] = alpha;
            st->mb_iters += 1;
        }
    }
    float au[3] = {0.f, 0.f, 0.f}, am[3] = {0.f, 0.f, 0.f}, at[3] = {0.f, 0.f, 0.f};
    for (int q = lane16; q < cnt; q += MB_LPR) {
        const bool first = q == lane16, second = q == lane16 + MB_LPR;
        const float2 e   = first ? e0 : second ? e1 : s.ell[(size_t)q * s.D + a];
        const int col    = __float_as_int(e.y);
        const float val  = e.x;
        const float4 uu  = first ? uu0 : second ? uu1 : ucur[col];
        au[0] = fmaf(val, uu.x, au[0]), au[1] = fmaf(val, uu.y, au[1]), au[2] = fmaf(val, uu.z, au[2]);
        if (it >= 0) {
            const float4 mm = first ? mm0 : second ? mm1 : mcur[col], tt = first ? tt0 : second ? tt1 : tprev[col];
            am[0] = fmaf(val, mm.x, am[0]), am[1] = fmaf(val, mm.y, am[1]), am[2] = fmaf(val, mm.z, am[2]);
            at[0] = fmaf(val, tt.x, at[0]), at[1] = fmaf(val, tt.y, at[1]), at[2] = fmaf(val, tt.z, at[2]);
        }
    }
#pragma unroll
    for (int c = 0; c < 3; ++c) au[c] = group16_sum(au[c]), am[c] = group16_sum(am[c]), at[c] = group16_sum(at[c]);
    float gpart = 0.f, dpart = 0.f;
    if (row_ok && lane16 == 0) {
        const float minv = jacobi_inv(s.diag[a]);
        float4 u = ucur[a], r = s.mb_r[a];
        float w[3] = {au[0], au[1], au[2]};
        if (it >= 0) {
            const float4 m = mcur[a], tp = tprev[a], p = s.mb_p[a], sv = s.mb_s[a], wv = s.mb_w[a];
            float4 x = s.mb_x[a];
            const float4 tn = make_float4(fmaf(beta, tp.x, m.x), fmaf(beta, tp.y, m.y), fmaf(beta, tp.z, m.z), 0.f);
            const float4 pn = make_float4(fmaf(beta, p.x, u.x), fmaf(beta, p.y, u.y), fmaf(beta, p.z, u.z), 0.f);
            const float4 sn = make_float4(fmaf(beta, sv.x, wv.x), fmaf(beta, sv.y, wv.y), fmaf(beta, sv.z, wv.z), 0.f);
            u = make_float4(fmaf(-alpha, tn.x, u.x), fmaf(-alpha, tn.y, u.y), fmaf(-alpha, tn.z, u.z), 0.f);
            r = make_float4(fmaf(-alpha, sn.x, r.x), fmaf(-alpha, sn.y, r.y), fmaf(-alpha, sn.z, r.z), 0.f);
            x.x = fmaf(alpha, pn.x, x.x), x.y = fmaf(alpha, pn.y, x.y), x.z = fmaf(alpha, pn.z, x.z);
#pragma unroll
            for (int c = 0; c < 3; ++c) w[c] = au[c] - alpha * (am[c] + beta * at[c]);
            s.mb_t[cur][a] = tn, s.mb_p[a] = pn, s.mb_s[a] = sn, s.mb_x[a] = x, s.mb_r[a] = r, s.mb_u[nxt][a] = u;
        }
        s.mb_w[a]                     = make_float4(w[0], w[1], w[2], 0.f);
        s.mb_m[it >= 0 ? nxt : 0][a] = make_float4(minv * w[0], minv * w[1], minv * w[2], 0.f);
        gpart = fmaf(r.z, u.z, fmaf(r.y, u.y, r.x * u.x));
        dpart = fmaf(w[2], u.z, fmaf(w[1], u.y, w[0] * u.x));
    }
    gpart = wave_sum_all(gpart), dpart = wave_sum_all(dpart);
    __syncthreads();
    if ((threadIdx.x & 63) == 0) sh[0][threadIdx.x >> 6] = gpart, sh[1][threadIdx.x >> 6] = dpart;
    __syncthreads();
    if (threadIdx.x == 0) {
        const int slot = it >= 0 ? ((it + 1) & 1) : 0;
        s.mb_gpart[slot][blockIdx.x] = (sh[0][0] + sh[0][1]) + (sh[0][2] + sh[0][3]);
        s.mb_dpart[slot][blockIdx.x] = (sh[1][0] + sh[1][1]) + (sh[1][2] + sh[1][3]);
    }
}

__global__ __launch_bounds__(256) void pcg_mb_finish_kernel(SolveView s, SolveState* __restrict__ st) {
    if (st->mb_skip) return;
    const int a = blockIdx.x * blockDim.x + threadIdx.x;
    if (a < s.D) {
        const float4 x = s.mb_x[a];
        s.t[3 * a] += x.x, s.t[3 * a + 1] += x.y, s.t[3 * a + 2] += x.z;
    }
    if (a == 0) pcg_book_launch(st, st->mb_rz0, st->mb_iters, false);
}

void MbGraphCache::release() {
    for (int i = 0; i < used; ++i)
        if (e[i].exec) (void)hipGraphExecDestroy(e[i].exec);
    used = 0;
    if (capture) (void)hipStreamDestroy(capture), capture = nullptr;
}

static hipError_t launch_mb_range(const SolveView& s, SolveState* state, int it0, int it1, float pcg_tol,
                                  MbGraphCache* gc, hipStream_t st) {
    const int nb = solve_mb_blocks(s.D);
    auto direct = [&](hipStream_t q) {
        for (int it = it0; it < it1; ++it) pcg_mb_step_kernel<<<nb, 256, 0, q>>>(s, state, it, pcg_tol);
        return hipGetLastError();
    };
    if (!gc || gc->disabled || it1 - it0 < 4) return direct(st);
    MbGraphCache::Entry* hit = nullptr;
    for (int i = 0; i < gc->used && !hit; ++i) {
        MbGraphCache::Entry& c = gc->e[i];
        if (c.it0 == it0 && c.it1 == it1 && c.tol == pcg_tol && c.state == state && c.view.D == s.D && c.view.ell == s.ell)
            hit = &c;
    }
    if (!hit) {
        if (gc->used == (int)(sizeof(gc->e) / sizeof(gc->e[0]))) {
            for (int i = 0; i < gc->used; ++i)
                if (gc->e[i].exec) (void)hipGraphExecDestroy(gc->e[i].exec);
            gc->used = 0;
        }
        hipGraph_t g = nullptr;
        hipGraphExec_t exec = nullptr;
        bool ok = gc->capture || hipStreamCreateWithFlags(&gc->capture, hipStreamNonBlocking) == hipSuccess;
        ok      = ok && hipStreamBeginCapture(gc->capture, hipStreamCaptureModeThreadLocal) == hipSuccess;
        if (ok) {
            const hipError_t le = direct(gc->capture);
            const hipError_t ce = hipStreamEndCapture(gc->capture, &g);
            ok = le == hipSuccess && ce == hipSuccess && g && hipGraphInstantiate(&exec, g, nullptr, nullptr, 0) == hipSuccess;
            if (g) (void)hipGraphDestroy(g);
        }
        if (!ok) {
            (void)hipGetLastError();
            gc->disabled = true;
            return direct(st);
        }
        hit        = &gc->e[gc->used++];
        hit->it0 = it0, hit->it1 = it1, hit->tol = pcg_tol, hit->view = s, hit->state = state, hit->exec = exec;
    }
    return hipGraphLaunch(hit->exec, st);
}

static hipError_t launch_mb_pcg(const SolveView& s, SolveState* state, int max_iter, float pcg_tol, int* host_flag,
                                MbGraphCache* gc, hipStream_t st) {
    const int nb = solve_mb_blocks(s.D), nbu = (s.D + 255) / 256;
    pcg_mb_init_kernel<<<nbu, 256, 0, st>>>(s, state);
    pcg_mb_step_kernel<<<nb, 256, 0, st>>>(s, state, -1, pcg_tol);
    int chunk = 16;
    const int ci = gc ? std::min(gc->call++, 63) : 0;
    if (gc && host_flag && gc->pred[ci] > 0) chunk = std::max(8, (gc->pred[ci] + 4 + 7) & ~7);
    for (int it = 0; it < max_iter;) {
        const int end = host_flag ? std::min(max_iter, it + chunk) : max_iter;
        {
            const hipError_t e = launch_mb_range(s, state, it, end, pcg_tol, host_flag ? gc : nullptr, st);
            if (e != hipSuccess) return e;
            it = end;
        }
        if (host_flag && it < max_iter) {
            pcg_mb_step_kernel<<<nb, 256, 0, st>>>(s, state, it, pcg_tol);
            hipError_t e = hipMemcpyAsync(host_flag, &state->mb_done, 4 * sizeof(int), hipMemcpyDeviceToHost, st);
            if (e == hipSuccess) e = hipStreamSynchronize(st);
            if (e != hipSuccess) return e;
            if (gc) gc->pred[ci] = host_flag[3];
            if (*host_flag) break;
            ++it;
            chunk = 16;
        }
    }
    pcg_mb_finish_kernel<<<nbu, 256, 0, st>>>(s, state);
    return hipGetLastError();
}

#if defined(__HIP_DEVICE_COMPILE__) && !defined(__gfx950__) && !defined(__gfx942__) && !defined(__gfx90a__)
#error "pcg_team_kernel orders its stores with s_waitcnt vmcnt(0): gfx9 only (gfx10+ count stores in vscnt)"
#endif
constexpr int TEAM_W = 32;
constexpr int TEAM_NT = 1024;
constexpr int TEAM_E = 20;
constexpr int TEAM_E_TREG = 16;
constexpr int TEAM_K = 4;
constexpr int TEAM_ROUNDS = 257;
constexpr size_t TEAM_MIN_LDS = 82 * 1024;
constexpr long long TEAM_TICKS_FIRST = 2000000, TEAM_TICKS = 500000;
__host__ __device__ constexpr size_t team_words_per_round() { return (size_t)TEAM_K * 2 * 2 * TEAM_W; }
size_t solve_team_pcg_words() { return 3 * (size_t)TEAM_ROUNDS * team_words_per_round(); }

__device__ __forceinline__ unsigned xcc_id() { return __builtin_amdgcn_s_getreg((3 << 11) | 20) & 0xf; }

__device__ __forceinline__ void team_give_up(TeamCtl* ctl, int c, int* host_abort) {
    if (atomicExch(&ctl->abort[c], 1u) == 0u && host_abort) atomicAdd_system(host_abort, 1);
}

template <bool JOINT>
__device__ __forceinline__ bool team_wait(const unsigned long long* __restrict__ wr , unsigned round,
                                          float (&sum)[3], const unsigned* abort_flag, long long ticks, float* bc ,
                                          long long* prof = nullptr, int rank = 0) {
    if (threadIdx.x < 64) {
        const int lane = threadIdx.x;
        long long t0 = 0;
        unsigned long long w0 = 0, w1 = 0;
        bool good = true;
#ifdef DFA_PCG_PROFILE
        const long long c0_ = clock64();
        bool own_seen = false;
#endif
        for (unsigned spins = 0;; ++spins) {
            const unsigned long long* p = wr + (size_t)(spins < (unsigned)TEAM_K ? spins : 0u) * (4 * TEAM_W) + lane;
            if (spins < (unsigned)TEAM_K) {
                w0 = __hip_atomic_load(p, __ATOMIC_RELAXED, __HIP_MEMORY_SCOPE_WAVEFRONT);
                if (JOINT) w1 = __hip_atomic_load(p + 2 * TEAM_W, __ATOMIC_RELAXED, __HIP_MEMORY_SCOPE_WAVEFRONT);
            } else {
                w0 = __hip_atomic_load(p, __ATOMIC_RELAXED, __HIP_MEMORY_SCOPE_AGENT);
                if (JOINT) w1 = __hip_atomic_load(p + 2 * TEAM_W, __ATOMIC_RELAXED, __HIP_MEMORY_SCOPE_AGENT);
            }
            const bool ok = (unsigned)(w0 >> 32) == round && (!JOINT || lane >= TEAM_W || (unsigned)(w1 >> 32) == round);
#ifdef DFA_PCG_PROFILE
            if (prof) {
                const bool mine_ok = __builtin_amdgcn_readlane((int)ok, rank);
                if (mine_ok && !own_seen) own_seen = true, prof[0] += clock64() - c0_;
                prof[1] += 1;
            }
// ... 478 lines not shown
```

dynfu_amd/csrc/solve.hpp:

```cpp
#pragma once
#include <hip/hip_runtime.h>
#include <stdint.h>

namespace dfa {

struct SolveState {
    double initial_cost;
    double cost;
    double final_cost;
    double grad_first;
    int have_initial;
    int done;
    int gn_iters;
    int pcg_iters;
    int max_row_nnz;
    int overflow;
    int pcg_fallback;
    int split_iters;
    unsigned int split_ticket;
    int mb_done;
    int converged;
    int mb_skip, mb_iters;
    int weights_fresh;
    int gn_noop;
    int cost_stale;
    float mb_rz0, mb_gamma_prev[2], mb_alpha_prev[2];
    float amax;
    long long prof[8];
};

__host__ __device__ inline bool solve_rec_ids16(int k) { return k % 8 == 0; }
__host__ __device__ inline int solve_rec_words(int k) { return solve_rec_ids16(k) ? k + k / 2 + 4 : 2 * k + 4; }
__host__ __device__ inline int solve_rec_tail(int k) { return solve_rec_words(k) - 4; }

__device__ __forceinline__ void solve_mark_at_floor(SolveState* st) {
    if (st->weights_fresh) st->converged = 1;
    else if (!st->converged) st->converged = 2;
}

struct TeamCtl {
    unsigned int count[3];
    unsigned int abort[3];
    unsigned int finished[3];
    int iters[3];
    float rz0[3];
    unsigned int at_floor[3];
};

struct SolveView {
    int N, D, k, Dpad, ell_cap;
    int deterministic;
    const float* node_pos;
    const float* node_dq;
    const float* node_w;
    const float* canon;
    const float* live;
    int32_t* ridx;
    float* rw;
    float* rtau;
    float* rb;
    float* re;
    int32_t* reg_idx;
    int32_t* blk_hist;
    int32_t* node_ptr;
    uint32_t* node_list;
    float2* ell;
    int32_t* ell_cnt;
    float* diag;
    float* g;
    float* g_base;
    float* t_base;
    int32_t* pk_perm;
    int32_t* pk_perm2;
    float* pk_vals;
    uint16_t* pk_cols;
    float4 *mb_x, *mb_r, *mb_p, *mb_s, *mb_w, *mb_u[2], *mb_m[2], *mb_t[2];
    float *mb_gpart[2], *mb_dpart[2];
    TeamCtl* team_ctl;
    float2* team_mt;
    unsigned long long* team_words;
    int team_stride;
    float* t;
    float* huber;
    float* node_dq_out;
};

constexpr int SOLVE_TG_BLOCKS = 256;
hipError_t solve_build_graph(const SolveView& s, SolveState* state, unsigned int* ticket, int nticket, hipStream_t st);
hipError_t solve_transpose_graph(const int32_t* ridx, size_t total, int D, int32_t* blk_hist, int32_t* node_ptr,
                                 uint32_t* node_list, hipStream_t st);
int solve_residual_blocks(const SolveView& s);
hipError_t solve_linearise(const SolveView& s, SolveState* state, double* cost_partials, unsigned int* ticket,
                           int update_weights, int mode, float gn_tol, float tukey_offset, float psi_data,
                           float w_reg_sq, float huber_psi ,
                           long long* iters_total , hipStream_t st);
hipError_t solve_huber(const SolveView& s, float psi_reg, hipStream_t st);
hipError_t solve_reset(const SolveView& s, SolveState* state, unsigned int* ticket, int nticket, hipStream_t st);
hipError_t solve_assemble(const SolveView& s, SolveState* state, int save_base , float w_reg_sq,
                          hipStream_t st);
hipError_t solve_regradient(const SolveView& s, SolveState* state, hipStream_t st);
int solve_pcg_max_nodes();
__host__ __device__ inline int solve_mb_rows_per_block() { return 16; }
__host__ __device__ inline int solve_mb_blocks(int D) { return (D + 15) / 16; }
struct MbGraphCache {
    struct Entry {
        int it0 = 0, it1 = 0;
        float tol = 0.f;
        SolveView view;
        const SolveState* state = nullptr;
        hipGraphExec_t exec = nullptr;
    };
    Entry e[24];
    int used = 0;
    int pred[64] = {};
    int call     = 0;
    hipStream_t capture = nullptr;
    bool disabled = false;
    void release();
};

struct TeamPcg {
    TeamCtl* ctl    = nullptr;
    int* host_abort = nullptr;
    unsigned epoch  = 1;
    long launches   = 0;
    bool disabled   = false;
};
bool solve_team_pcg_fits(int D);
int solve_team_pcg_rounds();
size_t solve_team_pcg_words();

bool solve_pcg_is_async(const SolveView& s, const TeamPcg* team, int max_iter);
hipError_t solve_pcg(const SolveView& s, SolveState* state, int max_iter, float pcg_tol, int* host_flag ,
                     MbGraphCache* graphs , TeamPcg* team , hipEvent_t main_done,
                     hipStream_t st);
hipError_t solve_count_noop(SolveState* state, int n, hipStream_t st);

}
```

Before: 1599 frames/s.

## Pack per-node entry stream for assembly and share translation loads in linearise

Builds a node-major entry array during graph transposition that stores each residual row's index, active weight, 16-bit neighbour ids and weights contiguously. The assemble kernel streams these entries with software prefetch instead of chasing row records through node_list, so its reads become coalesced and less indirect. Linearise now loads the per-row graph and node translations once and shares them with the Tukey weight computation. The max linearise block count is raised to 8192, with a looped reduction over the partials. The cost is extra memory and a write pass for the entry array, and the per-row record write is skipped outside the dev A/B build.

Result: no change. 1596 frames/s (-0.2%).

```diff
diff --git a/dynfu_amd/csrc/capi.cpp b/dynfu_amd/csrc/capi.cpp
--- a/dynfu_amd/csrc/capi.cpp
+++ b/dynfu_amd/csrc/capi.cpp
@@ -881,6 +881,7 @@
     A(blk_hist, D * (dfa::SOLVE_TG_BLOCKS + 1));
     A(node_ptr, D + 1);
     A(node_list, R * k);
+    A(node_ent, (R * k + 1) * (size_t)(dfa::solve_entry_words(k) / 4));
     A(ell, D * s->ell_cap);
     A(ell_cnt, D);
     A(diag, D);
@@ -934,7 +935,7 @@
     if (rc == DFA_OK) rc = plan_alloc(s, &s->iters_total, 1);
     if (rc == DFA_OK && hipMemset(s->iters_total, 0, sizeof(long long)) != hipSuccess) rc = DFA_ERR_HIP;
     if (rc == DFA_OK && hipHostMalloc((void**)&s->host_flag, 4 * sizeof(int), hipHostMallocDefault) != hipSuccess) s->host_flag = nullptr;
-    if (rc == DFA_OK) rc = plan_alloc(s, &s->cost_partials, std::max<size_t>((R + 255) / 256 + 1, 1024) + 1024);
+    if (rc == DFA_OK) rc = plan_alloc(s, &s->cost_partials, (size_t)2 * dfa::SOLVE_LIN_MAX_BLOCKS);
     if (rc == DFA_OK) rc = plan_alloc(s, &s->ticket, 64);
     if (rc == DFA_OK && hipMemset(s->ticket, 0, 64 * sizeof(unsigned int)) != hipSuccess)
         rc = fail(DFA_ERR_HIP, "hipMemset (ticket)");
diff --git a/dynfu_amd/csrc/solve.hip b/dynfu_amd/csrc/solve.hip
--- a/dynfu_amd/csrc/solve.hip
+++ b/dynfu_amd/csrc/solve.hip
@@ -52,10 +52,8 @@
     blk_hist[(size_t)TG_BLOCKS * D + i] = run;
 }
 
-__global__ __launch_bounds__(1024) void tg_fill_kernel(const int32_t* __restrict__ ridx, size_t total, int D,
-                                                       const int32_t* __restrict__ blk_base ,
-                                                       int32_t* __restrict__ node_ptr, uint32_t* __restrict__ node_list) {
-    extern __shared__ int32_t cursor[];
+__device__ __forceinline__ void tg_cursors(const int32_t* __restrict__ blk_base , int D,
+                                           int32_t* __restrict__ node_ptr, int32_t* cursor) {
     __shared__ int32_t wave_tot[16];
     __shared__ int32_t carry_sh;
     const int lane = threadIdx.x & 63, wave = threadIdx.x >> 6;
@@ -78,6 +76,13 @@
         __syncthreads();
     }
     if (blockIdx.x == 0 && threadIdx.x == 0) node_ptr[D] = carry_sh;
+}
+
+__global__ __launch_bounds__(1024) void tg_fill_kernel(const int32_t* __restrict__ ridx, size_t total, int D,
+                                                       const int32_t* __restrict__ blk_base ,
+                                                       int32_t* __restrict__ node_ptr, uint32_t* __restrict__ node_list) {
+    extern __shared__ int32_t cursor[];
+    tg_cursors(blk_base, D, node_ptr, cursor);
     const size_t chunk = (total + TG_BLOCKS - 1) / TG_BLOCKS;
     const size_t beg = chunk * blockIdx.x, end = min(beg + chunk, total);
     for (size_t e = beg + threadIdx.x; e < end; e += blockDim.x) {
@@ -103,27 +108,26 @@
     }
 }
 
-template <int K>
-__device__ __forceinline__ float tukey_weight(const SolveView& s, size_t v, float tukey_offset, float psi_data) {
+template <int K, bool OWN_T>
+__device__ __forceinline__ float tukey_weight(const SolveView& s, size_t v, const int (&n)[K], const float (&w)[K], const float (&tx)[K],
+                                              const float (&ty)[K], const float (&tz)[K], float tukey_offset, float psi_data) {
     const f3 c = mk3(s.canon[3 * v], s.canon[3 * v + 1], s.canon[3 * v + 2]);
     DQ sum     = dq_identity();
-    int n[K];
-    float w[K];
-    load_row_graph<K>(s, v, n, w);
 #pragma unroll
     for (int h = 0; h < K; h += 4) {
-        float tx[4], ty[4], tz[4];
+        float ux[4], uy[4], uz[4];
         DQ q[4];
 #pragma unroll
         for (int jj = 0; jj < 4; ++jj) {
             const int nn = n[h + jj] >= 0 ? n[h + jj] : 0;
-            tx[jj] = s.t[3 * nn], ty[jj] = s.t[3 * nn + 1], tz[jj] = s.t[3 * nn + 2];
-            q[jj]  = dq_load(s.node_dq + 8 * (size_t)nn);
+            if (OWN_T) ux[jj] = s.t[3 * nn], uy[jj] = s.t[3 * nn + 1], uz[jj] = s.t[3 * nn + 2];
+            else ux[jj] = tx[h + jj], uy[jj] = ty[h + jj], uz[jj] = tz[h + jj];
+            q[jj] = dq_load(s.node_dq + 8 * (size_t)nn);
         }
 #pragma unroll
         for (int jj = 0; jj < 4; ++jj) {
             if (n[h + jj] >= 0) {
-                const DQ cur = dq_mul(dq_from_translation(tx[jj], ty[jj], tz[jj]), q[jj]);
+                const DQ cur = dq_mul(dq_from_translation(ux[jj], uy[jj], uz[jj]), q[jj]);
                 sum          = dq_mul(sum, dq_scale(cur, w[h + jj]));
             }
         }
@@ -169,7 +173,7 @@
 };
 
 constexpr int LIN_SHARDS     = 32;
-constexpr int LIN_MAX_BLOCKS = 1024;
+constexpr int LIN_MAX_BLOCKS = SOLVE_LIN_MAX_BLOCKS;
 
 template <int K>
 __global__ __launch_bounds__(256) void linearise_kernel(SolveView s, SolveState* __restrict__ st,
@@ -195,29 +199,31 @@
     double c       = 0.0;
     float amax     = 0.f;
     for (size_t r = (size_t)blockIdx.x * blockDim.x + threadIdx.x; r < R; r += (size_t)gridDim.x * blockDim.x) {
+        constexpr bool SHARE_T = K <= 4;
+        int n[K];
+        float w[K], tx[K], ty[K], tz[K];
+        load_row_graph<K>(s, r, n, w);
+        auto load_t = [&]() {
+#pragma unroll
+            for (int j = 0; j < K; ++j) {
+                const int nn = n[j] >= 0 ? n[j] : 0;
+                tx[j] = s.t[3 * nn], ty[j] = s.t[3 * nn + 1], tz[j] = s.t[3 * nn + 2];
+            }
+        };
+        if (SHARE_T) load_t();
         float tau;
         if (a.update_weights) {
-            tau       = r < (size_t)s.N ? tukey_weight<K>(s, r, a.tukey_offset, a.psi_data) : a.w_reg_sq;
+            tau       = r < (size_t)s.N ? tukey_weight<K, !SHARE_T>(s, r, n, w, tx, ty, tz, a.tukey_offset, a.psi_data) : a.w_reg_sq;
             s.rtau[r] = tau;
         } else {
             tau = s.rtau[r];
         }
-        float sx = 0.f, sy = 0.f, sz = 0.f;
-        {
-            int n[K];
-            float w[K], tx[K], ty[K], tz[K];
-            load_row_graph<K>(s, r, n, w);
-#pragma unroll
-            for (int j = 0; j < K; ++j) {
-                const int nn = n[j] >= 0 ? n[j] : 0;
-                tx[j] = s.t[3 * nn], ty[j] = s.t[3 * nn + 1], tz[j] = s.t[3 * nn + 2];
-            }
-            float wm = 0.f;
-#pragma unroll
-            for (int j = 0; j < K; ++j)
-                if (n[j] >= 0) sx += w[j] * tx[j], sy += w[j] * ty[j], sz += w[j] * tz[j], wm = fmaxf(wm, fabsf(w[j]));
-            amax = fmaxf(amax, tau * wm * wm);
-        }
+        if (!SHARE_T) load_t();
+        float sx = 0.f, sy = 0.f, sz = 0.f, wm = 0.f;
+#pragma unroll
+        for (int j = 0; j < K; ++j)
+            if (n[j] >= 0) sx += w[j] * tx[j], sy += w[j] * ty[j], sz += w[j] * tz[j], wm = fmaxf(wm, fabsf(w[j]));
+        amax = fmaxf(amax, tau * wm * wm);
         const float ex = s.rb[3 * r] - sx, ey = s.rb[3 * r + 1] - sy, ez = s.rb[3 * r + 2] - sz;
         *(float4*)(s.re + r * (size_t)solve_rec_words(s.k) + solve_rec_tail(s.k)) = make_float4(ex, ey, ez, tau);
         c += (double)tau * ((double)ex * ex + (double)ey * ey + (double)ez * ez);
@@ -256,17 +262,19 @@
     __shared__ double smx[256];
     double acc = 0.0, mx = 0.0;
     {
-        constexpr int Q = LIN_MAX_BLOCKS / 256;
-        double cq[Q], mq[Q];
-#pragma unroll
-        for (int q = 0; q < Q; ++q) {
-            const unsigned int i = min(threadIdx.x + 256u * q, gridDim.x - 1);
-            cq[q] = __hip_atomic_load(&cost_partials[i], __ATOMIC_RELAXED, __HIP_MEMORY_SCOPE_AGENT);
-            mq[q] = a.update_weights ? __hip_atomic_load(&cost_partials[LIN_MAX_BLOCKS + i], __ATOMIC_RELAXED, __HIP_MEMORY_SCOPE_AGENT) : 0.0;
-        }
-#pragma unroll
-        for (int q = 0; q < Q; ++q)
-            if (threadIdx.x + 256u * q < gridDim.x) acc += cq[q], mx = fmax(mx, mq[q]);
+        constexpr int Q = 8;
+        for (unsigned int q0 = 0; 256u * q0 < gridDim.x; q0 += Q) {
+            double cq[Q], mq[Q];
+#pragma unroll
+            for (int q = 0; q < Q; ++q) {
+                const unsigned int i = min(threadIdx.x + 256u * (q0 + q), gridDim.x - 1);
+                cq[q] = __hip_atomic_load(&cost_partials[i], __ATOMIC_RELAXED, __HIP_MEMORY_SCOPE_AGENT);
+                mq[q] = a.update_weights ? __hip_atomic_load(&cost_partials[LIN_MAX_BLOCKS + i], __ATOMIC_RELAXED, __HIP_MEMORY_SCOPE_AGENT) : 0.0;
+            }
+#pragma unroll
+            for (int q = 0; q < Q; ++q)
+                if (threadIdx.x + 256u * (q0 + q) < gridDim.x) acc += cq[q], mx = fmax(mx, mq[q]);
+        }
     }
     sm[threadIdx.x] = acc, smx[threadIdx.x] = mx;
     __syncthreads();
@@ -343,6 +351,7 @@
         }
         s.rb[3 * r + 0] = s.rb[3 * r + 1] = s.rb[3 * r + 2] = 0.f;
     }
+    if (!kDevAB) return;
     float* rec = s.re + r * (size_t)solve_rec_words(k);
     if (wide) {
         float4* rec4 = reinterpret_cast<float4*>(rec);
@@ -377,6 +386,52 @@
 #pragma unroll
     for (int j = 0; j < K; ++j)
         if (j < k) rec[j] = __int_as_float(ids[j]), rec[k + j] = ws[j];
+}
+
+template <int K>
+__device__ __forceinline__ void write_entry(const SolveView& s, size_t pos, uint32_t e) {
+    constexpr int EW = solve_entry_words(K);
+    const uint32_t r = e / (uint32_t)s.k;
+    const int slot   = (int)(e - r * (uint32_t)s.k);
+    int n[K];
+    float w[K];
+    load_row_graph<K>(s, r, n, w);
+    float wa = 0.f;
+#pragma unroll
+    for (int j = 0; j < K; ++j) wa = (j == slot) ? w[j] : wa;
+    uint32_t wd[EW] = {};
+    wd[0] = r, wd[1] = __float_as_uint(wa);
+#pragma unroll
+    for (int j = 0; j < K / 2; ++j) {
+        const uint32_t lo = n[2 * j] < 0 ? 0xffffu : (uint32_t)n[2 * j], hi = n[2 * j + 1] < 0 ? 0xffffu : (uint32_t)n[2 * j + 1];
+        wd[2 + j]         = (lo & 0xffffu) | (hi << 16);
+    }
+#pragma unroll
+    for (int j = 0; j < K; ++j) wd[2 + K / 2 + j] = __float_as_uint(w[j]);
+    uint4* out = s.node_ent + pos * (EW / 4);
+#pragma unroll
+    for (int q = 0; q < EW / 4; ++q) out[q] = make_uint4(wd[4 * q], wd[4 * q + 1], wd[4 * q + 2], wd[4 * q + 3]);
+}
+
+template <int K>
+__global__ __launch_bounds__(1024) void tg_fill_entries_kernel(SolveView s, size_t total) {
+    extern __shared__ int32_t cursor[];
+    tg_cursors(s.blk_hist, s.D, s.node_ptr, cursor);
+    const size_t chunk = (total + TG_BLOCKS - 1) / TG_BLOCKS;
+    const size_t beg = chunk * blockIdx.x, end = min(beg + chunk, total);
+    for (size_t e = beg + threadIdx.x; e < end; e += blockDim.x) {
+        const int n = s.ridx[e];
+        if (n < 0) continue;
+        const int pos    = atomicAdd(&cursor[n], 1);
+        s.node_list[pos] = (uint32_t)e;
+        write_entry<K>(s, (size_t)pos, (uint32_t)e);
+    }
+}
+
+template <int K>
+__global__ __launch_bounds__(256) void fill_entries_kernel(SolveView s, size_t total) {
+    const size_t p = (size_t)blockIdx.x * blockDim.x + threadIdx.x;
+    if (p < total && p < (size_t)s.node_ptr[s.D]) write_entry<K>(s, p, s.node_list[p]);
 }
 
 
@@ -409,6 +464,365 @@
 }
 
 template <int K>
+struct Visit {
+    uint32_t row;
+    float wa;
+    int idx[K];
+    float w[K];
+};
+
+template <int K>
+struct EntryStream {
+    static constexpr int EW    = solve_entry_words(K);
+    static constexpr bool DEEP = K <= 4;
+    struct Raw {
+        uint4 q[EW / 4];
+    };
+    Raw cur, nxt;
+    float4 cur_t;
+    int p, end, last;
+
+    __device__ __forceinline__ Raw load(const SolveView& s, int pos) const {
+        const uint4* e = s.node_ent + (size_t)min(pos, last) * (EW / 4);
+        Raw r;
+#pragma unroll
+        for (int q = 0; q < EW / 4; ++q) r.q[q] = e[q];
+        return r;
+    }
+    __device__ __forceinline__ float4 tail(const SolveView& s, const Raw& r, int pos) const {
+        const size_t row = pos < end ? r.q[0].x : 0u;
+        return *(const float4*)(s.re + row * (size_t)solve_rec_words(s.k) + solve_rec_tail(s.k));
+    }
+    __device__ __forceinline__ void begin(const SolveView& s, int beg, int end_) {
+        end = end_, last = max(end_ - 1, beg), p = beg + (int)threadIdx.x;
+        cur = load(s, p);
+        if (DEEP) nxt = load(s, p + 256);
+        cur_t = tail(s, cur, p);
+    }
+    static __device__ __forceinline__ Visit<K> decode(const Raw& r) {
+        uint32_t wd[EW];
+#pragma unroll
+        for (int q = 0; q < EW / 4; ++q) wd[4 * q] = r.q[q].x, wd[4 * q + 1] = r.q[q].y, wd[4 * q + 2] = r.q[q].z, wd[4 * q + 3] = r.q[q].w;
+        Visit<K> v;
+        v.row = wd[0], v.wa = __uint_as_float(wd[1]);
+#pragma unroll
+        for (int j = 0; j < K / 2; ++j) {
+            const int lo = (int)(wd[2 + j] & 0xffffu), hi = (int)(wd[2 + j] >> 16);
+            v.idx[2 * j] = lo == 0xffff ? -1 : lo, v.idx[2 * j + 1] = hi == 0xffff ? -1 : hi;
+        }
+#pragma unroll
+        for (int j = 0; j < K; ++j) v.w[j] = __uint_as_float(wd[2 + K / 2 + j]);
+        return v;
+    }
+    template <class F>
+    __device__ __forceinline__ void run(const SolveView& s, F&& f) {
+        if (DEEP) {
+            for (; p < end; p += 256) {
+                const float4 nxt_t = tail(s, nxt, p + 256);
+                const Raw nn       = load(s, p + 512);
+                f(decode(cur), cur_t);
+                cur = nxt, cur_t = nxt_t, nxt = nn;
+            }
+        } else {
+            for (; p < end; p += 256) {
+                nxt = load(s, p + 256);
+                f(decode(cur), cur_t);
+                cur = nxt, cur_t = tail(s, cur, p + 256);
+            }
+        }
+    }
+};
+
+#ifdef DFA_PCG_PROFILE
+__device__ unsigned long long asm_tbuf[32768 * 8];
+extern "C" __attribute__((visibility("default"))) int dfa_dev_asm_timing(unsigned long long* out, int n) {
+    return (int)hipMemcpyFromSymbol(out, HIP_SYMBOL(asm_tbuf), sizeof(unsigned long long) * 8 * (size_t)n);
+}
+#endif
+
+template <int K>
+__global__ __launch_bounds__(256) void assemble_kernel(SolveView s, SolveState* __restrict__ st, int save_base, float amax_unset) {
+    __shared__ int key[HASH];
+    __shared__ long long val[2 * HASH];
+    __shared__ float gpart[4][3];
+    __shared__ int wave_cnt[4];
+    __shared__ int ovf;
+    const int a = blockIdx.x;
+    const int wave = threadIdx.x >> 6, lane = threadIdx.x & 63;
+#ifdef DFA_PCG_PROFILE
+    long long t0_ = clock64(), t1_, t2_, t3_, t4_;
+    const unsigned long long w0_ = wall_clock64();
+#endif
+    const int beg = s.node_ptr[a], end = s.node_ptr[a + 1];
+    const float amax_st = st->amax;
+    const int stop      = st->done | st->converged;
+    EntryStream<K> es;
+    es.begin(s, beg, end);
+    if (stop) return;
+    for (int i = threadIdx.x; i < HASH; i += 256) key[i] = -1, val[i] = val[i + HASH] = 0ll;
+    if (threadIdx.x == 0) ovf = 0;
+    __syncthreads();
+#ifdef DFA_PCG_PROFILE
+    t1_ = clock64();
+#endif
+
+    const FixedScale fx = fixed_scale_for_rows(solve_fixed_scale(amax_st > 0.f ? amax_st : amax_unset), end - beg);
+    float gx = 0.f, gy = 0.f, gz = 0.f, dsum = 0.f;
+    es.run(s, [&](const Visit<K>& v, const float4 et ) {
+        const float tw = et.w * v.wa;
+        gx += tw * et.x, gy += tw * et.y, gz += tw * et.z;
+        if (et.w != 0.f) {
+            uint32_t h0[K];
+            int k0[K];
+#pragma unroll
+            for (int j = 0; j < K; ++j) {
+                h0[j] = ((uint32_t)v.idx[j] * 2654435761u) >> (32 - 9);
+                k0[j] = key[h0[j]];
+            }
+#pragma unroll
+            for (int j = 0; j < K; ++j) {
+                const int b = v.idx[j];
+                if (b < 0) continue;
+                const float x = tw * v.w[j];
+                if (b == a) {
+                    dsum += x;
+                    continue;
+                }
+                if (k0[j] == b) {
+                    fixed_add(&val[h0[j]], x, fx.up);
+                    continue;
+                }
+                uint32_t h = h0[j];
+                int cur    = k0[j];
+#pragma unroll 1
+                for (int probes = 0;; ++probes) {
+                    if (cur == -1) cur = atomicCAS(&key[h], -1, b), cur = cur == -1 ? b : cur;
+                    if (cur == b) {
+                        fixed_add(&val[h], x, fx.up);
+                        break;
+                    }
+                    if (probes >= HASH) {
+                        ovf = 1;
+                        break;
+                    }
+                    h   = (h + 1) & HASH_MASK;
+                    cur = key[h];
+                }
+            }
+        }
+    });
+    dsum = wave_total(dsum);
+    if (lane == 0 && dsum != 0.f) {
+        uint32_t h = ((uint32_t)a * 2654435761u) >> (32 - 9);
+        for (int probes = 0; probes < HASH; ++probes, h = (h + 1) & HASH_MASK) {
+            const int cur = atomicCAS(&key[h], -1, a);
+            if (cur == -1 || cur == a) {
+                fixed_add(&val[h], dsum, fx.up);
+                break;
+            }
+        }
+    }
+#ifdef DFA_PCG_PROFILE
+    t2_ = clock64();
+#endif
+    gx = wave_total(gx), gy = wave_total(gy), gz = wave_total(gz);
+    if (lane == 0) gpart[wave][0] = gx, gpart[wave][1] = gy, gpart[wave][2] = gz;
+    __syncthreads();
+#ifdef DFA_PCG_PROFILE
+    t3_ = clock64();
+#endif
+    constexpr int PER_WAVE = HASH / 4;
+    constexpr int PER_LANE = PER_WAVE / 64;
+    int kk[PER_LANE];
+    float vv[PER_LANE];
+    int wcnt = 0;
+#pragma unroll
+    for (int i = 0; i < PER_LANE; ++i) {
+        const int hq = wave * PER_WAVE + 64 * i + lane;
+        kk[i]        = key[hq];
+        vv[i]        = (float)((double)(val[hq] - val[hq + HASH]) * fx.down);
+        wcnt += __popcll(__ballot(kk[i] >= 0));
+    }
+    if (lane == 0) wave_cnt[wave] = wcnt;
+    __syncthreads();
+    int pos0 = 0, total = 0;
+#pragma unroll
+    for (int w = 0; w < 4; ++w) {
+        pos0 += w < wave ? wave_cnt[w] : 0;
+        total += wave_cnt[w];
+    }
+#pragma unroll
+    for (int i = 0; i < PER_LANE; ++i) {
+        const uint64_t m = __ballot(kk[i] >= 0);
+        if (kk[i] >= 0) key[pos0 + __popcll(m & ((1ull << lane) - 1ull))] = kk[i];
+        pos0 += __popcll(m);
+    }
+    __syncthreads();
+    int rank[PER_LANE] = {};
+    for (int q = 0; q < total; ++q) {
+        const int kq = key[q];
+#pragma unroll
+        for (int i = 0; i < PER_LANE; ++i) rank[i] += kq < kk[i];
+    }
+    float diag = 0.f;
+#pragma unroll
+    for (int i = 0; i < PER_LANE; ++i) {
+        if (kk[i] < 0) continue;
+        if (rank[i] < s.ell_cap) s.ell[(size_t)rank[i] * s.D + a] = make_float2(vv[i], __int_as_float(kk[i]));
+        if (kk[i] == a) s.diag[a] = vv[i], diag = 1.f;
+    }
+    const bool has_diag = __syncthreads_or(diag != 0.f);
+    if (threadIdx.x == 0) {
+        s.ell_cnt[a] = min(total, s.ell_cap);
+        if (!has_diag) s.diag[a] = 0.f;
+#pragma unroll
+        for (int c = 0; c < 3; ++c) {
+            const float gc = (gpart[0][c] + gpart[1][c]) + (gpart[2][c] + gpart[3][c]);
+            s.g[3 * a + c] = gc;
+            if (save_base) s.g_base[3 * a + c] = gc, s.t_base[3 * a + c] = s.t[3 * a + c];
+        }
+        if (total > *(volatile int*)&st->max_row_nnz) atomicMax(&st->max_row_nnz, total);
+        if (total > s.ell_cap || ovf) st->overflow = 1;
+#ifdef DFA_PCG_PROFILE
+        t4_ = clock64();
+        if (a == 7 && !s.team_ctl) st->prof[6] = (t1_ - t0_) * 1000000 + (t2_ - t1_), st->prof[7] = (t3_ - t2_) * 1000000 + (t4_ - t3_);
+        if (a < 32768) {
+            unsigned long long* o = asm_tbuf + 8 * (size_t)a;
+            o[0] = w0_, o[1] = wall_clock64() - w0_, o[2] = (unsigned long long)(end - beg), o[3] = (unsigned long long)total;
+            o[4] = t1_ - t0_, o[5] = t2_ - t1_, o[6] = t3_ - t2_, o[7] = t4_ - t3_;
+        }
+#endif
+    }
+}
+
+constexpr int DET_SORT_MAX = 4096;
+
+__global__ __launch_bounds__(256) void sort_node_lists_kernel(const int32_t* __restrict__ node_ptr, uint32_t* __restrict__ node_list) {
+    __shared__ uint32_t buf[DET_SORT_MAX];
+    const int a = blockIdx.x, tid = threadIdx.x;
+    const int beg = node_ptr[a], len = node_ptr[a + 1] - beg;
+    if (len < 2 || len > DET_SORT_MAX) return;
+    int n2 = 1;
+    while (n2 < len) n2 <<= 1;
+    for (int i = tid; i < n2; i += 256) buf[i] = i < len ? node_list[beg + i] : 0xffffffffu;
+    __syncthreads();
+    for (int size = 2; size <= n2; size <<= 1)
+        for (int stride = size >> 1; stride > 0; stride >>= 1) {
+            for (int i = tid; i < n2 / 2; i += 256) {
+                const int lo = 2 * i - (i & (stride - 1)), hi = lo + stride;
+                const bool up = (lo & size) == 0;
+                const uint32_t x = buf[lo], y = buf[hi];
+                if ((x > y) == up) buf[lo] = y, buf[hi] = x;
+            }
+            __syncthreads();
+        }
+    for (int i = tid; i < len; i += 256) node_list[beg + i] = buf[i];
+}
+
+template <int K>
+__global__ __launch_bounds__(256) void assemble_det_kernel(SolveView s, SolveState* __restrict__ st, int save_base, float amax_unset) {
+    __shared__ int key[HASH];
+    __shared__ long long val[2 * HASH];
+    __shared__ float gpart[4][3], dpart[4];
+    __shared__ int ovf, nkeys;
+    const int a    = blockIdx.x;
+    const int wave = threadIdx.x >> 6, lane = threadIdx.x & 63;
+    const int beg = s.node_ptr[a], end = s.node_ptr[a + 1];
+    const float amax_st = st->amax;
+    const int stop      = st->done | st->converged;
+    EntryStream<K> es;
+    es.begin(s, beg, end);
+    if (stop) return;
+    for (int i = threadIdx.x; i < HASH; i += 256) key[i] = -1, val[i] = val[i + HASH] = 0ll;
+    if (threadIdx.x == 0) ovf = 0, nkeys = 0;
+    __syncthreads();
+    const FixedScale fx = fixed_scale_for_rows(solve_fixed_scale(amax_st > 0.f ? amax_st : amax_unset), end - beg);
+    float gx = 0.f, gy = 0.f, gz = 0.f, dsum = 0.f;
+    es.run(s, [&](const Visit<K>& v, const float4 et) {
+        const float tw = et.w * v.wa;
+        gx += tw * et.x, gy += tw * et.y, gz += tw * et.z;
+        if (et.w != 0.f) {
+#pragma unroll
+            for (int j = 0; j < K; ++j) {
+                const int b = v.idx[j];
+                if (b < 0) continue;
+                if (b == a) {
+                    dsum += tw * v.w[j];
+                    continue;
+                }
+                uint32_t h = ((uint32_t)b * 2654435761u) >> (32 - 9);
+                for (int probes = 0;; ++probes) {
+                    const int cur = atomicCAS(&key[h], -1, b);
+                    if (cur == -1 || cur == b) break;
+                    if (probes >= HASH) {
+                        ovf = 1;
+                        break;
+                    }
+                    h = (h + 1) & HASH_MASK;
+                }
+            }
+        }
+    });
+    es.begin(s, beg, end);
+    dsum = wave_total(dsum), gx = wave_total(gx), gy = wave_total(gy), gz = wave_total(gz);
+    if (lane == 0) dpart[wave] = dsum, gpart[wave][0] = gx, gpart[wave][1] = gy, gpart[wave][2] = gz;
+    __syncthreads();
+    const float dtot = (dpart[0] + dpart[1]) + (dpart[2] + dpart[3]);
+    if (threadIdx.x == 0 && dtot != 0.f) {
+        uint32_t h = ((uint32_t)a * 2654435761u) >> (32 - 9);
+        for (int probes = 0; probes < HASH; ++probes, h = (h + 1) & HASH_MASK)
+            if (key[h] == -1) {
+                key[h] = a;
+                break;
+            }
+    }
+    __syncthreads();
+    es.run(s, [&](const Visit<K>& v, const float4 et) {
+        if (et.w == 0.f) return;
+        const float tw = et.w * v.wa;
+#pragma unroll
+        for (int j = 0; j < K; ++j) {
+            const int b = v.idx[j];
+            if (b < 0 || b == a) continue;
+            uint32_t h = ((uint32_t)b * 2654435761u) >> (32 - 9);
+            for (int probes = 0; probes <= HASH && key[h] != b; ++probes) h = (h + 1) & HASH_MASK;
+            if (key[h] == b) fixed_add(&val[h], tw * v.w[j], fx.up);
+        }
+    });
+    __syncthreads();
+    int total = 0;
+    for (int i = threadIdx.x; i < HASH; i += 256) total += key[i] >= 0;
+    total = (int)wave_total((float)total);
+    if (lane == 0) atomicAdd(&nkeys, total);
+    __syncthreads();
+    total = nkeys;
+    bool has_diag = false;
+    for (int i = threadIdx.x; i < HASH; i += 256) {
+        const int kk = key[i];
+        if (kk < 0) continue;
+        int pos = 0;
+        for (int q = 0; q < HASH; ++q) pos += key[q] >= 0 && key[q] < kk;
+        const float vv = kk == a ? dtot : (float)((double)(val[i] - val[i + HASH]) * fx.down);
+        if (pos < s.ell_cap) s.ell[(size_t)pos * s.D + a] = make_float2(vv, __int_as_float(kk));
+        if (kk == a) s.diag[a] = vv, has_diag = true;
+    }
+    const bool any_diag = __syncthreads_or(has_diag);
+    if (threadIdx.x == 0) {
+        s.ell_cnt[a] = min(total, s.ell_cap);
+        if (!any_diag) s.diag[a] = 0.f;
+#pragma unroll
+        for (int c = 0; c < 3; ++c) {
+            const float gc = (gpart[0][c] + gpart[1][c]) + (gpart[2][c] + gpart[3][c]);
+            s.g[3 * a + c] = gc;
+            if (save_base) s.g_base[3 * a + c] = gc, s.t_base[3 * a + c] = s.t[3 * a + c];
+        }
+        if (total > *(volatile int*)&st->max_row_nnz) atomicMax(&st->max_row_nnz, total);
+        if (total > s.ell_cap || ovf) st->overflow = 1;
+    }
+}
+
+#ifdef DFA_DEV_AB
+template <int K>
 __device__ __forceinline__ float4 load_record(const SolveView& s, size_t r, int (&idx)[K], float (&w)[K]) {
     const float* rec = s.re + r * (size_t)solve_rec_words(s.k);
     if (s.k == K && (K % 8) == 0) {
@@ -460,15 +874,8 @@
     return make_float4(rec[2 * s.k], rec[2 * s.k + 1], rec[2 * s.k + 2], rec[2 * s.k + 3]);
 }
 
-#ifdef DFA_PCG_PROFILE
-__device__ unsigned long long asm_tbuf[32768 * 8];
-extern "C" __attribute__((visibility("default"))) int dfa_dev_asm_timing(unsigned long long* out, int n) {
-    return (int)hipMemcpyFromSymbol(out, HIP_SYMBOL(asm_tbuf), sizeof(unsigned long long) * 8 * (size_t)n);
-}
-#endif
-
 template <int K>
-__global__ __launch_bounds__(256) void assemble_kernel(SolveView s, SolveState* __restrict__ st, int save_base, float amax_unset) {
+__global__ __launch_bounds__(256) void assemble_records_kernel(SolveView s, SolveState* __restrict__ st, int save_base, float amax_unset) {
     __shared__ int key[HASH];
     __shared__ long long val[2 * HASH];
     __shared__ float gpart[4][3];
@@ -477,16 +884,9 @@
     if (st->done || st->converged) return;
     const int a = blockIdx.x;
     const int wave = threadIdx.x >> 6, lane = threadIdx.x & 63;
-#ifdef DFA_PCG_PROFILE
-    long long t0_ = clock64(), t1_, t2_, t3_, t4_;
-    const unsigned long long w0_ = wall_clock64();
-#endif
     for (int i = threadIdx.x; i < HASH; i += 256) key[i] = -1, val[i] = val[i + HASH] = 0ll;
     if (threadIdx.x == 0) ovf = 0;
     __syncthreads();
-#ifdef DFA_PCG_PROFILE
-    t1_ = clock64();
-#endif
 
     const int beg = s.node_ptr[a], end = s.node_ptr[a + 1];
     const FixedScale fx = fixed_scale_for_rows(solve_fixed_scale(st->amax > 0.f ? st->amax : amax_unset), end - beg);
@@ -554,15 +954,9 @@
             }
         }
     }
-#ifdef DFA_PCG_PROFILE
-    t2_ = clock64();
-#endif
     gx = wave_total(gx), gy = wave_total(gy), gz = wave_total(gz);
     if (lane == 0) gpart[wave][0] = gx, gpart[wave][1] = gy, gpart[wave][2] = gz;
     __syncthreads();
-#ifdef DFA_PCG_PROFILE
-    t3_ = clock64();
-#endif
     constexpr int PER_WAVE = HASH / 4;
     constexpr int PER_LANE = PER_WAVE / 64;
     int kk[PER_LANE];
@@ -615,44 +1009,12 @@
         }
         if (total > *(volatile int*)&st->max_row_nnz) atomicMax(&st->max_row_nnz, total);
         if (total > s.ell_cap || ovf) st->overflow = 1;
-#ifdef DFA_PCG_PROFILE
-        t4_ = clock64();
-        if (a == 7 && !s.team_ctl) st->prof[6] = (t1_ - t0_) * 1000000 + (t2_ - t1_), st->prof[7] = (t3_ - t2_) * 1000000 + (t4_ - t3_);
-        if (a < 32768) {
-            unsigned long long* o = asm_tbuf + 8 * (size_t)a;
-            o[0] = w0_, o[1] = wall_clock64() - w0_, o[2] = (unsigned long long)(end - beg), o[3] = (unsigned long long)total;
-            o[4] = t1_ - t0_, o[5] = t2_ - t1_, o[6] = t3_ - t2_, o[7] = t4_ - t3_;
-        }
-#endif
-    }
-}
-
-constexpr int DET_SORT_MAX = 4096;
-
-__global__ __launch_bounds__(256) void sort_node_lists_kernel(const int32_t* __restrict__ node_ptr, uint32_t* __restrict__ node_list) {
-    __shared__ uint32_t buf[DET_SORT_MAX];
-    const int a = blockIdx.x, tid = threadIdx.x;
-    const int beg = node_ptr[a], len = node_ptr[a + 1] - beg;
-    if (len < 2 || len > DET_SORT_MAX) return;
-    int n2 = 1;
-    while (n2 < len) n2 <<= 1;
-    for (int i = tid; i < n2; i += 256) buf[i] = i < len ? node_list[beg + i] : 0xffffffffu;
-    __syncthreads();
-    for (int size = 2; size <= n2; size <<= 1)
-        for (int stride = size >> 1; stride > 0; stride >>= 1) {
-            for (int i = tid; i < n2 / 2; i += 256) {
-                const int lo = 2 * i - (i & (stride - 1)), hi = lo + stride;
-                const bool up = (lo & size) == 0;
-                const uint32_t x = buf[lo], y = buf[hi];
-                if ((x > y) == up) buf[lo] = y, buf[hi] = x;
-            }
-            __syncthreads();
-        }
-    for (int i = tid; i < len; i += 256) node_list[beg + i] = buf[i];
-}
+    }
+}
+
 
 template <int K>
-__global__ __launch_bounds__(256) void assemble_det_kernel(SolveView s, SolveState* __restrict__ st, int save_base, float amax_unset) {
+__global__ __launch_bounds__(256) void assemble_det_records_kernel(SolveView s, SolveState* __restrict__ st, int save_base, float amax_unset) {
     __shared__ int key[HASH];
     __shared__ long long val[2 * HASH];
     __shared__ float gpart[4][3], dpart[4];
@@ -765,6 +1127,8 @@
         if (total > s.ell_cap || ovf) st->overflow = 1;
     }
 }
+
+#endif
 
 template <int NT, int R>
 __device__ __forceinline__ void stable_equal_runs(const int32_t* from, int32_t* to, const int32_t* cnt_of_row, const int* hist, int D) {
@@ -1373,8 +1737,13 @@
     const size_t lds = sizeof(int32_t) * (size_t)D;
     tg_count_kernel<<<TG_BLOCKS, 1024, lds, st>>>(s.ridx, total, D, s.blk_hist);
     tg_colscan_kernel<<<(D + 255) / 256, 256, 0, st>>>(s.blk_hist, D);
-    tg_fill_kernel<<<TG_BLOCKS, 1024, lds, st>>>(s.ridx, total, D, s.blk_hist, s.node_ptr, s.node_list);
-    if (s.deterministic) sort_node_lists_kernel<<<D, 256, 0, st>>>(s.node_ptr, s.node_list);
+    if (s.deterministic) {
+        tg_fill_kernel<<<TG_BLOCKS, 1024, lds, st>>>(s.ridx, total, D, s.blk_hist, s.node_ptr, s.node_list);
+        sort_node_lists_kernel<<<D, 256, 0, st>>>(s.node_ptr, s.node_list);
+        KDISPATCH(fill_entries_kernel, k, <<<(unsigned)((total + 255) / 256), 256, 0, st>>>(s, total));
+    } else {
+        KDISPATCH(tg_fill_entries_kernel, k, <<<TG_BLOCKS, 1024, lds, st>>>(s, total));
+    }
     return hipGetLastError();
 }
 
@@ -1405,6 +1774,13 @@
 
 hipError_t solve_assemble(const SolveView& s, SolveState* state, int save_base, float w_reg_sq, hipStream_t st) {
     const float amax_unset = std::max(1.0f, w_reg_sq);
+#ifdef DFA_DEV_AB
+    if (dev_env_int("DFA_ASSEMBLE_RECORDS", 0)) {
+        if (s.deterministic) KDISPATCH(assemble_det_records_kernel, s.k, <<<s.D, 256, 0, st>>>(s, state, save_base, amax_unset));
+        else KDISPATCH(assemble_records_kernel, s.k, <<<s.D, 256, 0, st>>>(s, state, save_base, amax_unset));
+        return hipGetLastError();
+    }
+#endif
     if (s.deterministic) KDISPATCH(assemble_det_kernel, s.k, <<<s.D, 256, 0, st>>>(s, state, save_base, amax_unset));
     else KDISPATCH(assemble_kernel, s.k, <<<s.D, 256, 0, st>>>(s, state, save_base, amax_unset));
     return hipGetLastError();
diff --git a/dynfu_amd/csrc/solve.hpp b/dynfu_amd/csrc/solve.hpp
--- a/dynfu_amd/csrc/solve.hpp
+++ b/dynfu_amd/csrc/solve.hpp
@@ -33,6 +33,9 @@
 __host__ __device__ inline int solve_rec_words(int k) { return solve_rec_ids16(k) ? k + k / 2 + 4 : 2 * k + 4; }
 __host__ __device__ inline int solve_rec_tail(int k) { return solve_rec_words(k) - 4; }
 
+__host__ __device__ constexpr int solve_entry_slots(int k) { return k <= 4 ? 4 : k <= 8 ? 8 : 16; }
+__host__ __device__ constexpr int solve_entry_words(int k) { return (2 + solve_entry_slots(k) / 2 + solve_entry_slots(k) + 3) & ~3; }
+
 __device__ __forceinline__ void solve_mark_at_floor(SolveState* st) {
     if (st->weights_fresh) st->converged = 1;
     else if (!st->converged) st->converged = 2;
@@ -64,6 +67,7 @@
     int32_t* blk_hist;
     int32_t* node_ptr;
     uint32_t* node_list;
+    uint4* node_ent;
     float2* ell;
     int32_t* ell_cnt;
     float* diag;
@@ -85,6 +89,7 @@
     float* node_dq_out;
 };
 
+constexpr int SOLVE_LIN_MAX_BLOCKS = 8192;
 constexpr int SOLVE_TG_BLOCKS = 256;
 hipError_t solve_build_graph(const SolveView& s, SolveState* state, unsigned int* ticket, int nticket, hipStream_t st);
 hipError_t solve_transpose_graph(const int32_t* ridx, size_t total, int D, int32_t* blk_hist, int32_t* node_ptr,
```
